# funkelab/cellulus

Hardware: AMD Instinct MI355X
Metric: train crops/sec (U-Net fwd+bwd + OCE loss + Adam) (higher is better)
Workload: dtype f32 (exact 3xbf16 operand split, 6 products, f32 accumulate)

## Files before the change

### cellulus_amd/_clx.py

```python

import ctypes
import os
from ctypes import POINTER, Structure, c_char_p, c_double, c_int, c_longlong, c_size_t, c_void_p

import torch

_HERE = os.path.dirname(os.path.abspath(__file__))
LIB_PATH = os.path.join(_HERE, "libclx.so")


class ClxError(RuntimeError):
    """A libclx entry point returned a negative status."""


class ClxSrc(Structure):

    _fields_ = [
        ("ptr", c_void_p),
        ("C", c_int),
        ("ld", c_int),
        ("D", c_int),
        ("H", c_int),
        ("W", c_int),
        ("oz", c_int),
# ... 6 lines not shown


class ClxPackJob(Structure):

    _fields_ = [("w", c_void_p), ("wp", c_void_p), ("cout", c_int), ("cin", c_int), ("taps", c_int),
                ("cin_pad", c_int), ("cout_pad", c_int), ("mode", c_int)]


class ClxConvDesc(Structure):

    _fields_ = [
        ("nsrc", c_int),
        ("src", ClxSrc * 2),
        ("B", c_int),
        ("ID", c_int),
        ("IH", c_int),
        ("IW", c_int),
        ("KD", c_int),
        ("KH", c_int),
        ("KW", c_int),
        ("PD", c_int),
        ("PH", c_int),
        ("PW", c_int),
        ("N", c_int),
        ("wpack", c_void_p),
        ("bias", c_void_p),
        ("relu", c_int),
        ("mask", c_void_p),
        ("ld_mask", c_int),
        ("out", c_void_p),
        ("ld_out", c_int),
        ("accumulate", c_int),
        ("algo", c_int),
        ("workspace", c_void_p),
        ("workspace_bytes", c_size_t),
        ("vcache", c_void_p),
        ("vcache_valid", c_int),
        ("c_real", c_int),
        ("dy_vcache", c_void_p),
        ("gate_out", c_void_p),
        ("ld_gate", c_int),
        ("mask_bits", c_void_p),
        ("ld_mask_bits", c_int),
        ("det_turns", c_void_p),
        ("adjoint", c_int),
        ("pool_out", c_void_p),
        ("ld_pool", c_int),
        ("tile_list", c_void_p),
        ("tile_count", c_int),
        ("precision", c_int),
        ("wplanes", c_void_p),
        ("aplanes", c_void_p),
        ("aplanes_valid", c_int),
        ("dyplanes", c_void_p),
        ("dyplanes_valid", c_int),
        ("out_planes", c_void_p),
        ("out_colsum", c_void_p),
    ]


_P = c_void_p
_I = c_int
_LL = c_longlong
_D = c_double

PROTOTYPES = {
    "clx_last_error": (c_char_p, []),
    "clx_abi_version": (_I, []),
    "clx_device_count": (_I, []),
    "clx_profile_enable": (_I, [_I]),
    "clx_profile_read": (_I, [_I, POINTER(c_double), POINTER(c_double), POINTER(c_double)]),
    "clx_profile_clock": (_I, [POINTER(c_double), POINTER(c_double), _I]),
    "clx_conv_fwd": (_I, [POINTER(ClxConvDesc), _P]),
    "clx_conv_wgrad": (_I, [POINTER(ClxConvDesc), _P, _I, _P, _P, _P]),
    "clx_chain64_fwd": (_I, [_P, _I, _LL, _P, _P, _P, _I, _P, _I, _P, _P, _I, _I, _P, _I, _P, _I, _P]),
    "clx_chain64_bwd": (_I, [_P, _I, _I, _P, _I, _P, _I, _I, _LL, _P, _P, _P, _I, _P, _P, _P, _P, _P]),
    "clx_pack_weights": (_I, [_P, _P, _I, _I, _I, _I, _I, _I, _P]),
    "clx_pack_weights_batch": (_I, [_P, _I, _LL, _P]),
    "clx_unpack_wgrad": (_I, [_P, _P, _I, _I, _I, _I, _I, _P]),
    "clx_unpack_wgrad_wino": (_I, [_P, _P, _I, _I, _I, _I, _I, _I, _I, _P]),
    "clx_conv_workspace_bytes": (c_size_t, [POINTER(ClxConvDesc), _I]),
    "clx_conv_vcache_bytes": (c_size_t, [POINTER(ClxConvDesc), _I]),
    "clx_conv_sp_covers": (_I, [POINTER(ClxConvDesc), _I]),
    "clx_planes_bytes": (c_size_t, [_LL, _I]),
    "clx_split_planes": (_I, [_P, _LL, _LL, _I, _P, _P]),
    "clx_join_planes": (_I, [_P, _LL, _I, _P, _LL, _P]),
    "clx_gemm_planes": (_I, [_P, _P, _I, _I, _I, _P, _I, _P, _I, _P]),
    "clx_wgrad_planes": (_I, [_P, _P, _LL, _I, _I, _P, _I, _P]),
    "clx_conv_fused_applicable": (_I, [POINTER(ClxConvDesc)]),
    "clx_conv_fused_workspace_bytes": (c_size_t, [POINTER(ClxConvDesc)]),
    "clx_planar_to_pixel": (_I, [_P, _P, _I, _I, _LL, _I, _P]),
    "clx_pixel_to_planar": (_I, [_P, _P, _I, _I, _LL, _I, _P]),
    "clx_depth_to_space": (_I, [_P, _I, _P, _I, _I, _I, _I, _I, _I, _I, _I, _I, _P]),
    "clx_space_to_depth": (_I, [_P, _I, _P, _I, _I, _I, _I, _I, _I, _I, _I, _I, _P]),
    "clx_subpixel_split_weights": (_I, [_P, _P, _P] + [_I] * 10 + [_P]),
    "clx_subpixel_fold_grads": (_I, [_P, _P, _P] + [_I] * 10 + [_P]),
    "clx_maxpool_fwd": (_I, [_P, _P, _I, _I, _I, _I, _I, _I, _I, _I, _P]),
    "clx_changed_rows_workspace": (c_size_t, [_I, _I, _I, _I]),
    "clx_changed_rows": (_I, [_P, _P, _I, _I, _I, _I, _I, _I, _I, _I, _I, _P, _P, _LL, _P, _P]),
    "clx_changed_tiles": (_I, [_P, _I, _I, _I, _I, _I, _I, _I, _I, _I, _I, _I, _P, _P, _LL, _P]),
    "clx_grey_rows": (_I, [_P, _I, _I, _I, _I, _I, _P, _LL, _P, _P, _I, _I, _P, _I, _P]),
    "clx_conv_first_dgrad": (_I, [_P, _I, _P, _I, _I, _I, _I, _I, _I, _I, _P, _P]),
    "clx_gather_rows": (_I, [_P, _I, _P, _LL, _I, _P, _I, _P]),
    "clx_scatter_rows": (_I, [_P, _I, _P, _LL, _I, _P, _I, _P]),
    "clx_broadcast_rows": (_I, [_P, _LL, _P, _I, _P]),
    "clx_maxpool_bwd": (_I, [_P, _P, _P, _P] + [_I] * 7 + [_P] + [_I] * 8 + [_P]),
    "clx_upsample_bwd": (_I, [_P] + [_I] * 8 + [_P, _P] + [_I] * 8 + [_P]),
    "clx_gather_add_fwd": (_I, [_P, _P, _P, _I, _I, _I, _I, _I, _I, _P, _P]),
    "clx_gather_add_bwd": (_I, [_P, _P, _P, _I, _I, _I, _I, _I, _I, _P, _P]),
    "clx_oce_loss_fwd_bwd": (_I, [_P, _P, _P, _P, _LL, _I, ctypes.c_float, ctypes.c_float, ctypes.c_float, _P]),
    "clx_conv_wgrad_turns_bytes": (c_size_t, [POINTER(ClxConvDesc)]),
    "clx_colsum_scratch_bytes": (c_size_t, [_I]),
    "clx_colsum_ordered": (_I, [_P, _I, _LL, _I, _P, _P, _P]),
    "clx_oce_pairs_det_scratch_bytes": (c_size_t, [_I, _I, _LL]),
    "clx_oce_pairs_fused_det": (_I, [_P, _P, _P, _P, _P, _I, _I, _I, _I, _I, _I, ctypes.c_float, ctypes.c_float, _P, _P]),
    "clx_oce_pairs_fused": (_I, [_P, _P, _P, _P, _P, _I, _I, _I, _I, _I, _I, ctypes.c_float, ctypes.c_float, _P]),
    "clx_sample_pairs": (_I, [_P, _P, _P, _I, _I, _I, _I, _I, _I, POINTER(c_int), ctypes.c_ulonglong,
                              ctypes.c_ulonglong, _P]),
    "clx_adam_step": (_I, [_P, _P, _P, _P, _LL, _D, _D, _D, _D, _D, _I, _P]),
    "clx_adam_step_guarded": (_I, [_P, _P, _P, _P, _LL, _D, _D, _D, _D, _D, _I, _P, _P]),
    "clx_noise_stats": (_I, [_P, _P, _I, _I, _LL, _P]),
    "clx_noise_inject": (_I, [_P, _P, _P, _I, _I, _LL, ctypes.c_float, _P]),
    "clx_zero_many": (_I, [POINTER(_P), POINTER(_LL), _I, _P]),
    "clx_gather_rows_f64": (_I, [_P, _P, _LL, _I, _P, _P]),
    "clx_rows_extent_f64": (_I, [_P, _LL, _I, _P, _P]),
    "clx_noise_stats_minmax": (_I, [_P, _P, _I, _I, _LL, _P, _I, _P]),
    "clx_ms_prepare_workspace": (c_size_t, [_LL]),
    "clx_ms_prepare": (_I, [_P, _P, _D, _I, _I, _I, _I, _P, _P, _P, _P, _P]),
    "clx_ms_prepare_f32": (_I, [_P, _P, _D, _I, _I, _I, _I, _P, _P, _P, _P, _P]),
    "clx_ms_iterate": (_I, [_P, _I, _P, _I, _I, _D, _I, _P, _P, _P, _P]),
    "clx_ms_iterate_grid": (_I, [_P, _I, _P, POINTER(c_double), _D, _I, _I, _I, _P, _I, _I, _D, _I,
                                 _P, _P, _P, _P]),
    "clx_ms_assign": (_I, [_P, _P, _I, _P, _I, _I, _P, _P]),
    "clx_ms_assign_grid": (_I, [_P, _P, _I, _P, _I, _I, _P, _P, POINTER(c_double), _D, _I, _I, _I, _P, _P]),
    "clx_ms_assign_cells": (_I, [_P, _P, _I, _P, _I, _I, _P, _P, POINTER(c_double), _D, _I, _I, _I, _P, _P]),
    "clx_ms_assign_dense": (_I, [_P, _P, _I, _I, _P, _P, POINTER(c_double), _D, _I, _I, _I, _P, _I, _I, _I, _I, _P, _P]),
    "clx_ms_dedup_centers": (_I, [_P, _P, _I, _I, _D, _P, POINTER(_I)]),
    "clx_sample_offsets_mt19937": (_I, [_P, POINTER(_I), _I, _I, _LL, _P, POINTER(_I)]),
    "clx_elastic_crop_workspace": (c_size_t, [_I, POINTER(c_int), _I]),
    "clx_elastic_crop": (_I, [_P, _I, _I, _I, _I, POINTER(c_int), POINTER(c_int), POINTER(c_int), ctypes.c_float, _I, _I,
                              _P, _P, _P, _P, _P, _P]),
    "clx_ms_bucket_workspace": (c_size_t, [_I, _LL]),
    "clx_ms_bucket": (_I, [_P, _I, _I, POINTER(c_double), _D, _I, _I, _I, _P, _P, _P, _P]),
    "clx_offset_magnitude": (_I, [_P, _P, _I, _LL, _P]),
    "clx_gaussian_filter_f64": (_I, [_P, _P, _P, _I, _I, _I, _P, _I, _P]),
    "clx_negate_f64": (_I, [_P, _P, _LL, _P]),
    "clx_peak_local_max": (_I, [_P, _I, _I, _I, _P, _P, _I, _P, _P]),
    "clx_greedy_cluster": (_I, [_P, _P, _I, _I, _I, _D, _I, _D, _I, _P, _P, _P, _P]),
    "clx_cc_workspace": (c_size_t, [_LL]),
    "clx_cc_label_filter": (_I, [_P, _P, _I, _I, _I, _I, _P, _P, _P]),
    "clx_edt_workspace": (c_size_t, [_LL]),
    "clx_edt_sq": (_I, [_P, _P, _I, _I, _I, _I, _P, _P]),
    "clx_grow_shrink": (_I, [_P, _I, _I, _I, _I, _I, _P, _P]),
    "clx_minmax_f64": (_I, [_P, _LL, _P, _P]),
    "clx_histogram_f64": (_I, [_P, _LL, _P, _I, _P, _P]),
    "clx_minmax_f32": (_I, [_P, _LL, _P, _P]),
    "clx_histogram_f32": (_I, [_P, _LL, _P, _I, _P, _P]),
    "clx_inst_stats": (_I, [_P, _P, _I, _I, _I, _I, _I, _P, _P, _P]),
    "clx_inst_histogram": (_I, [_P, _P, _I, _LL, _P, _I, _P, _I, _P, _P]),
    "clx_inst_refine": (_I, [_P, _P, _I, _I, _I, _I, _I, _P, _P, _P, _P, _P, _I, _P, _P]),
    "clx_lz4_decompress": (_LL, [_P, _LL, _P, _LL]),
    "clx_blosclz_decompress": (_LL, [_P, _LL, _P, _LL]),
    "clx_blosc_compress_bound": (_LL, [_LL]),
    "clx_blosc_compress_lz4": (_LL, [_P, _LL, _I, _I, _P, _LL]),
    "clx_unshuffle_bytes": (_I, [_P, _P, _LL, _I]),
    "clx_label_presence": (_I, [_P, _LL, _I, _P, _P, _P]),
# ... 90 lines not shown
```

### cellulus_amd/csrc/clx_common.h

```cpp
#pragma once
#include <hip/hip_runtime.h>
#include <hip/hip_ext.h>
#include <stdint.h>
#include <stdio.h>
#include <stdarg.h>
#include "../../include/clx.h"

void clx_set_error(const char* fmt, ...);

#define CLX_REQUIRE(cond, ...)                \
  do {                                        \
    if (!(cond)) {                            \
      clx_set_error(__VA_ARGS__);             \
      return CLX_ERR_ARG;                     \
    }                                         \
  } while (0)

#define CLX_CHECK_LAUNCH(name)                                           \
  do {                                                                   \
    hipError_t e__ = hipGetLastError();                                  \
    if (e__ != hipSuccess) {                                             \
      clx_set_error("%s: launch failed: %s", name, hipGetErrorString(e__)); \
      return CLX_ERR_LAUNCH;                                             \
    }                                                                    \
  } while (0)

typedef float f32x4 __attribute__((ext_vector_type(4)));
typedef float f32x16 __attribute__((ext_vector_type(16)));

struct FastDiv {
  uint32_t m, l, d;
};
static inline FastDiv make_fastdiv(uint32_t d) {
  FastDiv f;
  f.d = d;
  uint32_t l = 0;
  while ((1ull << l) < d) ++l;
  f.l = l;
  f.m = (uint32_t)(((1ull << 32) * ((1ull << l) - d)) / d + 1);
  return f;
}
__device__ __forceinline__ uint32_t fdiv(uint32_t n, const FastDiv& f) {
  return (__umulhi(f.m, n) + n) >> f.l;
}

__device__ __forceinline__ int xcd_remap(int bid, int nblocks) {
  const int q = nblocks >> 3, r = nblocks & 7;
  const int xcd = bid & 7, idx = bid >> 3;
  const int base = (xcd < r) ? xcd * (q + 1) : r * (q + 1) + (xcd - r) * q;
  return base + idx;
}

static inline int cdiv(long long a, long long b) { return (int)((a + b - 1) / b); }

bool clx_smallc_applicable(const clx_conv_desc* d);
int clx_smallc_fwd(const clx_conv_desc* d, hipStream_t st);
int clx_smallc_wgrad(const clx_conv_desc* d, const float* dy, int ld_dy, float* dwpack,
                     float* dbias, hipStream_t st);

int clx_igemm_launch(const clx_conv_desc* d, int batch, long long bs_in, long long bs_w,
                     long long bs_out, hipStream_t st);
int clx_wgrad_launch(const clx_conv_desc* d, const float* dy, int ld_dy, float* dwpack, float* dbias,
                     int batch, long long bs_x, long long bs_dy, long long bs_out, hipStream_t st);
bool clx_sp_fwd_rule(const clx_conv_desc* d);
bool clx_sp_wgrad_rule(const clx_conv_desc* d);
bool clx_sp_applicable(const clx_conv_desc* d);
bool clx_wino_sp(const clx_conv_desc* d);
int clx_sp_launch(const void* A, const void* B, int M, int N, int K, long long rows_a, int batch, long long bs_a, long long bs_b,
                  long long bs_out, const clx_conv_desc* ep, hipStream_t st);
int clx_sp_clock_read(double* shader_ticks, double* wall_ticks, int reset);
int clx_sp_split(const float* x, long long ld, long long rows, int K, void* planes, float* colsum, int nreal, hipStream_t st);
int clx_sp_wgrad_launch(const void* dy_planes, const void* x_planes, long long rows, int N, int C, int batch, long long bs_dy,
                        long long bs_x, long long bs_out, float* dw, int ld_dw, hipStream_t st);
int clx_wino_fwd(const clx_conv_desc* d, hipStream_t st);
int clx_wino_wgrad(const clx_conv_desc* d, const float* dy, int ld_dy, float* dwpack, float* dbias,
                   hipStream_t st);
int clx_wino_pack(const float* w, float* wp, int cout, int cin, int cin_pad, int cout_pad, int dgrad, int tile,
                  int ksize, int kd, hipStream_t st);

int clx_wino_fused_fwd(const clx_conv_desc* d, hipStream_t st);

bool clx_prof_enabled();
void clx_prof_events(int kind, double flops, hipEvent_t* e0, hipEvent_t* e1);
#define CLX_LAUNCH_TIMED(kernel, grid, block, st, e0, e1, ...) \
  hipExtLaunchKernelGGL(kernel, grid, block, 0, st, e0, e1, 0, __VA_ARGS__)
#define CLX_LAUNCH_KIND(kind, kernel, grid, block, lds, st, ...)                              \
  do {                                                                                        \
    hipEvent_t e0__ = nullptr, e1__ = nullptr;                                                \
    if (clx_prof_enabled()) clx_prof_events(kind, 0.0, &e0__, &e1__);                         \
    hipExtLaunchKernelGGL(kernel, grid, block, lds, st, e0__, e1__, 0, __VA_ARGS__);          \
  } while (0)
```

### cellulus_amd/csrc/conv_igemm.hip

```cpp
#include "clx_common.h"
#include <stdlib.h>

#ifdef IG_STAMP
__device__ unsigned long long g_stamps[8 * 32768];
extern "C" int clx_debug_stamps(unsigned long long* host, int n) {
  return hipMemcpyFromSymbol(host, HIP_SYMBOL(g_stamps), sizeof(unsigned long long) * n) == hipSuccess ? 0 : 1;
}
#define STAMP(k) do { if (threadIdx.x == 0 && blockIdx.y == 0 && blockIdx.x < 32768) g_stamps[blockIdx.x * 8 + (k)] = wall_clock64(); } while (0)
#else
#define STAMP(k) do {} while (0)
#endif

__device__ unsigned long long g_clk_ticks[2];
extern "C" int clx_profile_clock(double* shader_ticks, double* wall_ticks_100mhz, int reset) {
  unsigned long long h[2] = {0ull, 0ull};
  if (hipMemcpyFromSymbol(h, HIP_SYMBOL(g_clk_ticks), sizeof(h)) != hipSuccess) {
    clx_set_error("clx_profile_clock: copy failed");
    return CLX_ERR_LAUNCH;
  }
  double sc = 0.0, sw = 0.0;
  if (clx_sp_clock_read(&sc, &sw, reset) != CLX_OK) {
    clx_set_error("clx_profile_clock: copy failed");
    return CLX_ERR_LAUNCH;
  }
// ... 459 lines not shown
          float x = val[j][e];
          if (p.mask) x = (p.mask[(size_t)mrow[j] * p.ld_mask + n + e] > 0.f) ? x : 0.f;
          dst[e] = x;
        }
      }
    }
  }
  STAMP(3);
  if (clk_block) { atomicAdd(&g_clk_ticks[0], clock64() - clk_c0); atomicAdd(&g_clk_ticks[1], wall_clock64() - clk_w0); }
}

}

static const float* zero_buffer() {
  static const float* cache[64] = {nullptr};
  int dev = 0;
  if (hipGetDevice(&dev) != hipSuccess || dev < 0 || dev >= 64) return nullptr;
  if (cache[dev] == nullptr) {
    void* ptr = nullptr;
    if (hipGetSymbolAddress(&ptr, HIP_SYMBOL(g_zero16)) != hipSuccess) return nullptr;
    cache[dev] = (const float*)ptr;
  }
  return cache[dev];
}

static int conv_validate(const clx_conv_desc* d, const char* who) {
  CLX_REQUIRE(d != nullptr, "%s: null descriptor", who);
  CLX_REQUIRE(d->nsrc == 1 || d->nsrc == 2, "%s: nsrc must be 1 or 2", who);
  CLX_REQUIRE(d->B > 0 && d->ID > 0 && d->IH > 0 && d->IW > 0, "%s: bad extent", who);
  const int K[3] = {d->KD, d->KH, d->KW};
  const int P[3] = {d->PD, d->PH, d->PW};
  const int I[3] = {d->ID, d->IH, d->IW};
  for (int i = 0; i < 3; ++i) {
    CLX_REQUIRE(K[i] >= 1 && K[i] <= 3, "%s: kernel extent must be 1, 2 or 3", who);
    CLX_REQUIRE(P[i] >= 0 && P[i] < K[i], "%s: padding must be < kernel extent", who);
    CLX_REQUIRE(I[i] + 2 * P[i] - K[i] + 1 > 0, "%s: input smaller than kernel", who);
  }
  for (int s = 0; s < d->nsrc; ++s) {
    const clx_src& S = d->src[s];
    CLX_REQUIRE(S.ptr != nullptr, "%s: null source %d", who, s);
    CLX_REQUIRE(S.C > 0 && S.C % 4 == 0 && S.ld % 4 == 0 && S.ld >= S.C,
                "%s: source channels/ld must be multiples of 4 (C=%d ld=%d)", who, S.C, S.ld);
    CLX_REQUIRE(((uintptr_t)S.ptr & 15) == 0, "%s: source pointer must be 16-byte aligned", who);
    CLX_REQUIRE(S.fz >= 1 && S.fy >= 1 && S.fx >= 1, "%s: upsample factors >= 1", who);
    CLX_REQUIRE(S.oz >= 0 && S.oy >= 0 && S.ox >= 0, "%s: negative crop", who);
    CLX_REQUIRE((d->ID - 1 + S.oz) / S.fz < S.D && (d->IH - 1 + S.oy) / S.fy < S.H &&
                    (d->IW - 1 + S.ox) / S.fx < S.W,
                "%s: source %d smaller than the logical input", who, s);
  }
  const long long M = (long long)d->B * (d->ID + 2 * d->PD - d->KD + 1) *
                      (d->IH + 2 * d->PH - d->KH + 1) * (d->IW + 2 * d->PW - d->KW + 1);
  CLX_REQUIRE(M < (1ll << 31), "%s: too many output pixels", who);
  return CLX_OK;
}

static void fill_params(const clx_conv_desc* d, ConvP& p) {
  p.nsrc = d->nsrc;
  for (int s = 0; s < 2; ++s) {
    const clx_src& S = d->src[s < d->nsrc ? s : 0];
    p.src[s] = SrcP{S.ptr, S.C, S.ld, S.D, S.H, S.W, S.oz, S.oy, S.ox, S.fz, S.fy, S.fx};
  }
  p.B = d->B; p.ID = d->ID; p.IH = d->IH; p.IW = d->IW;
  p.KD = d->KD; p.KH = d->KH; p.KW = d->KW;
  p.PD = d->PD; p.PH = d->PH; p.PW = d->PW;
  p.OD = d->ID + 2 * d->PD - d->KD + 1;
  p.OH = d->IH + 2 * d->PH - d->KH + 1;
  p.OW = d->IW + 2 * d->PW - d->KW + 1;
  p.N = d->N;
  p.M = d->B * p.OD * p.OH * p.OW;
  p.Ctot = d->src[0].C + (d->nsrc == 2 ? d->src[1].C : 0);
  p.Ktot = p.Ctot * d->KD * d->KH * d->KW;
  p.dOW = make_fastdiv(p.OW); p.dOH = make_fastdiv(p.OH); p.dOD = make_fastdiv(p.OD);
  p.wpack = d->wpack; p.bias = d->bias; p.mask = d->mask; p.out = d->out;
  p.gate_out = d->gate_out; p.ld_gate = d->ld_gate; p.mask_bits = d->mask_bits; p.ld_mask_bits = d->ld_mask_bits;
  p.relu = d->relu; p.ld_mask = d->ld_mask; p.ld_out = d->ld_out;
  p.accumulate = d->accumulate;
  p.bs_in = p.bs_w = p.bs_out = 0;
  p.flush_every = 0;
}

extern "C" int clx_conv_fwd(const clx_conv_desc* d, clx_stream stream) {
  int rc = conv_validate(d, "clx_conv_fwd");
  if (rc) return rc;
  CLX_REQUIRE(d->wpack && d->out, "clx_conv_fwd: null wpack/out");
  CLX_REQUIRE(d->N > 0 && d->ld_out >= d->N, "clx_conv_fwd: bad N/ld_out");
  CLX_REQUIRE(((uintptr_t)d->wpack & 15) == 0, "clx_conv_fwd: wpack must be 16-byte aligned");
  CLX_REQUIRE(d->mask == nullptr || (d->ld_mask >= d->N && d->ld_mask % 4 == 0 &&
                                     ((uintptr_t)d->mask & 15) == 0),
              "clx_conv_fwd: mask must be 16-byte aligned with ld_mask %% 4 == 0 and >= N");
  CLX_REQUIRE(d->ld_out % 4 == 0 && ((uintptr_t)d->out & 15) == 0,
              "clx_conv_fwd: out must be 16-byte aligned with ld_out %% 4 == 0");
  CLX_REQUIRE(d->gate_out == nullptr || (d->relu && d->ld_out % 32 == 0 && d->ld_gate * 32 >= d->ld_out),
              "clx_conv_fwd: gate_out needs relu, ld_out %% 32 == 0 and ld_gate >= ld_out / 32");
  CLX_REQUIRE(d->mask_bits == nullptr || (d->mask == nullptr && d->ld_mask_bits * 32 >= d->N),
              "clx_conv_fwd: mask_bits replaces mask and needs ld_mask_bits >= ceil(N / 32)");
  CLX_REQUIRE(d->algo == CLX_ALGO_DIRECT || d->algo == CLX_ALGO_WINOGRAD || d->algo == CLX_ALGO_WINOGRAD4 ||
                  d->algo == CLX_ALGO_WINOGRAD4_FUSED,
              "clx_conv_fwd: bad algo");
  CLX_REQUIRE((d->out_planes == nullptr && d->out_colsum == nullptr && !d->aplanes_valid) ||
                  (d->algo == CLX_ALGO_DIRECT && d->aplanes != nullptr && clx_sp_applicable(d)),
              "clx_conv_fwd: out_planes / out_colsum / aplanes_valid need the split-precision 1x1 product "
              "(clx_conv_sp_covers, wplanes and aplanes)");
  if (d->algo == CLX_ALGO_WINOGRAD4_FUSED) return clx_wino_fused_fwd(d, (hipStream_t)stream);
  if (d->algo != CLX_ALGO_DIRECT) return clx_wino_fwd(d, (hipStream_t)stream);
  CLX_REQUIRE(d->pool_out == nullptr && d->tile_list == nullptr && !d->adjoint,
              "clx_conv_fwd: pool_out / tile_list / adjoint need a Winograd algorithm (algo = %d)", d->algo);
  if (clx_smallc_applicable(d) && d->mask == nullptr && d->mask_bits == nullptr && d->gate_out == nullptr) {
    clx_smallc_fwd(d, (hipStream_t)stream);
    CLX_CHECK_LAUNCH("clx_conv_fwd(small-channel)");
    return CLX_OK;
  }
  rc = clx_igemm_launch(d, 1, 0, 0, 0, (hipStream_t)stream);
  if (rc) return rc;
  CLX_CHECK_LAUNCH("clx_conv_fwd");
  return CLX_OK;
}

int clx_igemm_launch(const clx_conv_desc* d, int batch, long long bs_in, long long bs_w,
                     long long bs_out, hipStream_t st) {
  if (batch == 1 && d->aplanes != nullptr && clx_sp_applicable(d)) {
    const clx_src& S = d->src[0];
    const long long M = (long long)d->B * d->ID * d->IH * d->IW;
    if (!d->aplanes_valid) {
      const int rc = clx_sp_split(S.ptr, S.ld, M, S.C, d->aplanes, nullptr, 0, st);
      if (rc) return rc;
    }
    return clx_sp_launch(d->aplanes, d->wplanes, (int)M, d->N, S.C, M, 1, 0, 0, 0, d, st);
  }
  ConvP p;
  fill_params(d, p);
  p.zeros = zero_buffer();
  CLX_REQUIRE(p.zeros != nullptr, "clx_conv_fwd: cannot resolve the device zero buffer");
  p.bs_in = bs_in; p.bs_w = bs_w; p.bs_out = bs_out;
  static const int flush_env = getenv("CLX_IGEMM_FLUSH") ? atoi(getenv("CLX_IGEMM_FLUSH")) : 2;
  p.flush_every = flush_env > 0 ? flush_env : 0;
  const bool wide = d->N > 64 && (double)(cdiv(d->N, 128) * 128) / d->N <= 1.2;
  hipEvent_t e0 = nullptr, e1 = nullptr;
  if (clx_prof_enabled())
    clx_prof_events(wide ? CLX_PROF_IGEMM_WIDE : CLX_PROF_IGEMM_NARROW, 2.0 * p.M * p.N * p.Ktot * batch, &e0, &e1);
  static const bool fast_env = getenv("CLX_IGEMM_FAST") == nullptr || atoi(getenv("CLX_IGEMM_FAST")) != 0;
  int fast = fast_env && (long long)p.N * p.Ktot < (1ll << 30) ? 1 : 0;
  const bool padded = d->PD != 0 || d->PH != 0 || d->PW != 0;
  for (int s = 0; s < d->nsrc && fast; ++s) {
    const clx_src& S = d->src[s];
    const long long floats = (long long)d->B * S.D * S.H * S.W * S.ld;
    if (S.C % BK != 0 || floats >= (padded ? (1ll << 29) : (1ll << 30))) fast = 0;
  }
  if (fast && padded) fast = 2;
  static const bool dbg = getenv("CLX_IGEMM_DEBUG") != nullptr;
  if (dbg) fprintf(stderr, "igemm fast=%d wide=%d M=%d N=%d K=%d batch=%d pad=%d%d%d k=%d%d%d nsrc=%d C0=%d\n", (int)fast, (int)wide, p.M, p.N, p.Ktot, batch, d->PD, d->PH, d->PW, d->KD, d->KH, d->KW, d->nsrc, d->src[0].C);
  if (wide) {
    p.nbm = cdiv(p.M, 128); p.nbn = cdiv(p.N, 128);
    if (fast == 1) CLX_LAUNCH_TIMED((conv_igemm_kernel<128, 128, 2, 2, 1>), dim3(p.nbm * p.nbn, batch), dim3(256), st, e0, e1, p);
    else if (fast == 2) CLX_LAUNCH_TIMED((conv_igemm_kernel<128, 128, 2, 2, 2>), dim3(p.nbm * p.nbn, batch), dim3(256), st, e0, e1, p);
    else CLX_LAUNCH_TIMED((conv_igemm_kernel<128, 128, 2, 2>), dim3(p.nbm * p.nbn, batch), dim3(256), st, e0, e1, p);
  } else {
    p.nbm = cdiv(p.M, 128); p.nbn = cdiv(p.N, 64);
    if (fast == 1) CLX_LAUNCH_TIMED((conv_igemm_kernel<128, 64, 4, 1, 1>), dim3(p.nbm * p.nbn, batch), dim3(256), st, e0, e1, p);
    else if (fast == 2) CLX_LAUNCH_TIMED((conv_igemm_kernel<128, 64, 4, 1, 2>), dim3(p.nbm * p.nbn, batch), dim3(256), st, e0, e1, p);
    else CLX_LAUNCH_TIMED((conv_igemm_kernel<128, 64, 4, 1>), dim3(p.nbm * p.nbn, batch), dim3(256), st, e0, e1, p);
  }
  return CLX_OK;
}
```

### cellulus_amd/csrc/conv_smallc.hip

```cpp
#include "clx_common.h"

namespace {

struct SmallP {
  const float* x;
  int ld_x, B, D, H, W;
  int oz, oy, ox;
  int ID, IH, IW, KD, KH, KW, PD, PH, PW, OD, OH, OW;
  int N, M, taps;
  FastDiv dOW, dOH, dOD;
  const float* wpack;
  const float* bias;
  float* out;
  int ld_out, relu;
  const float* dy;
  int ld_dy;
  float* dwp;
  float* dbias;
  int tiles_per_block;
  int RX, items;
  FastDiv dRX;
};

constexpr int PT = 64;
constexpr int MAX_TAPS = 27;

template <int PTILE>
__device__ __forceinline__ void stage_patch(const SmallP& p, int m0, float* Xs) {
  static_assert(256 % PTILE == 0, "a thread keeps one pixel of the tile");
  const int K4 = p.taps;
  const int pl = threadIdx.x % PTILE;
  const uint32_t m = (uint32_t)(m0 + pl);
  const bool live = m < (uint32_t)p.M;
  const uint32_t q1 = fdiv(m, p.dOW);
  const int ox = (int)(m - q1 * p.OW);
  const uint32_t q2 = fdiv(q1, p.dOH);
  const int oy = (int)(q1 - q2 * p.OH);
  const uint32_t q3 = fdiv(q2, p.dOD);
  const int oz = (int)(q2 - q3 * p.OD);
  const int b = (int)q3;
  int tx = 0, ty = 0, tz = 0;
  {
    const int tap = threadIdx.x / PTILE;
    tx = tap % p.KW; ty = (tap / p.KW) % p.KH; tz = tap / (p.KW * p.KH);
  }
  constexpr int STEP = 256 / PTILE;
  for (int tap = threadIdx.x / PTILE; tap < K4; tap += STEP) {
    f32x4 v = {0.f, 0.f, 0.f, 0.f};
    const int lz = oz + tz - p.PD, ly = oy + ty - p.PH, lx = ox + tx - p.PW;
    if (live && (unsigned)lz < (unsigned)p.ID && (unsigned)ly < (unsigned)p.IH && (unsigned)lx < (unsigned)p.IW) {
      const long long pix = (((long long)b * p.D + lz + p.oz) * p.H + ly + p.oy) * p.W + lx + p.ox;
      v = *reinterpret_cast<const f32x4*>(p.x + pix * p.ld_x);
    }
    *reinterpret_cast<f32x4*>(&Xs[(pl * K4 + tap) * 4]) = v;
    tx += STEP;
    while (tx >= p.KW) { tx -= p.KW; if (++ty == p.KH) { ty = 0; ++tz; } }
  }
}

template <int NG>
__global__ __launch_bounds__(256) void conv_smallc_fwd_kernel(const SmallP p) {
  constexpr int PL = 256 / NG;
  constexpr int PPT = PT / PL;
  extern __shared__ float smem[];
  const int K = p.taps * 4;
  float* Ws = smem;
  float* Xs = smem + K * NG * 4;
  const int n0 = blockIdx.y * NG * 4;
  const int ng = threadIdx.x % NG, pl = threadIdx.x / NG;
  __shared__ int used_channels;
  if (threadIdx.x == 0) used_channels = 0;
  __syncthreads();
  int mine_used = 0;
  for (int idx = threadIdx.x; idx < K * NG * 4; idx += 256) {
    const int n = idx / K, k = idx % K;
    const float wv = (n0 + n < p.N) ? p.wpack[(size_t)(n0 + n) * K + k] : 0.f;
    Ws[k * NG * 4 + n] = wv;
    if (wv != 0.f) mine_used |= 1 << (k & 3);
  }
  if (mine_used) atomicOr(&used_channels, mine_used);
  const int n = n0 + ng * 4;
  f32x4 bv = {0.f, 0.f, 0.f, 0.f};
  if (p.bias && n < p.N) {
#pragma unroll
    for (int e = 0; e < 4; ++e) bv[e] = (n + e < p.N) ? p.bias[n + e] : 0.f;
  }
  for (int t = 0; t < p.tiles_per_block; ++t) {
    const int m0 = (blockIdx.x * p.tiles_per_block + t) * PT;
    if (m0 >= p.M) break;
    __syncthreads();
    stage_patch<PT>(p, m0, Xs);
    __syncthreads();
    f32x4 acc[PPT];
#pragma unroll
    for (int i = 0; i < PPT; ++i) acc[i] = bv;
    const int used = used_channels;
    for (int c = 0; c < 4; ++c) {
// ... 85 lines not shown
      }
    } else {
#pragma unroll
      for (int a = 0; a < MT; ++a) {
        if (a < ntap) {
          const int tap = tap0 + a;
          const int lz = oz + tap / (p.KW * p.KH) - p.PD, ly = oy + (tap / p.KW) % p.KH - p.PH, lx = ox + tap % p.KW - p.PW;
          f32x4 xv = {0.f, 0.f, 0.f, 0.f};
          if ((unsigned)lz < (unsigned)p.ID && (unsigned)ly < (unsigned)p.IH && (unsigned)lx < (unsigned)p.IW) {
            const long long pix = (((long long)b * p.D + lz + p.oz) * p.H + ly + p.oy) * p.W + lx + p.ox;
            xv = *reinterpret_cast<const f32x4*>(p.x + pix * p.ld_x);
          }
#pragma unroll
          for (int c = 0; c < 4; ++c) acc[a][c] += xv[c] * dyv;
        }
      }
    }
  }
  __syncthreads();
#pragma unroll
  for (int a = 0; a < MT; ++a) {
    if (a < ntap) {
#pragma unroll
      for (int c = 0; c < 4; ++c)
#pragma unroll
        for (int e = 0; e < 4; ++e) atomicAdd(&red[(a * 4 + c) * NT + g * 4 + e], acc[a][c][e]);
    }
  }
#pragma unroll
  for (int e = 0; e < 4; ++e) atomicAdd(&red[ntap * 4 * NT + g * 4 + e], bsum[e]);
  __syncthreads();
  for (int i = threadIdx.x; i < ntap * 4 * NT; i += 256) {
    const int nl = i % NT, c = (i / NT) & 3, tap = tap0 + i / (4 * NT);
    if (n0 + nl < p.N) atomicAdd(p.dwp + ((size_t)tap * p.N + n0 + nl) * 4 + c, red[i]);
  }
  if (p.dbias && tap0 == 0)
    for (int i = threadIdx.x; i < NT; i += 256)
      if (n0 + i < p.N) atomicAdd(p.dbias + n0 + i, red[ntap * 4 * NT + i]);
}

struct Run {
  int ox0, m0;
  long long base;
};

__device__ __forceinline__ Run decode_run(const SmallP& p, uint32_t item) {
  const uint32_t q1 = fdiv(item, p.dRX);
  const int rx = (int)(item - q1 * p.RX);
  const uint32_t q2 = fdiv(q1, p.dOH);
  const int oy = (int)(q1 - q2 * p.OH);
  const uint32_t q3 = fdiv(q2, p.dOD);
  const int oz = (int)(q2 - q3 * p.OD);
  const int b = (int)q3;
  Run r;
  r.ox0 = rx * 4;
  r.m0 = ((b * p.OD + oz) * p.OH + oy) * p.OW + r.ox0;
  r.base = (((long long)b * p.D + oz + p.oz) * p.H + oy + p.oy) * p.W + r.ox0 + p.ox;
  return r;
}

template <int KD>
struct GreyLane {
  static constexpr int R = KD * 3, NP = R * 6, TAPS = R * 3;
  int px, cq, col;
  long long poff;
  __device__ __forceinline__ GreyLane(const SmallP& p) {
    const int lane = threadIdx.x & 63;
    px = lane >> 4; cq = lane & 15;
    const int l = lane < NP ? lane : 0;
    const int r = l / 6;
    col = l - r * 6;
    const int tz = r / 3, ty = r - tz * 3;
    poff = ((long long)tz * p.H + ty) * p.W;
  }
  __device__ __forceinline__ float load_patch(const SmallP& p, const Run& r) const {
    const int c = r.ox0 + col < p.IW ? col : p.IW - 1 - r.ox0;
    return p.x[(r.base + poff + c) * p.ld_x];
  }
  __device__ __forceinline__ float tap(float pv, int row, int tx) const {
    return __shfl(pv, row * 6 + tx + px, 64);
  }
};

template <int KD>
__global__ __launch_bounds__(256) void conv_grey_fwd_kernel(const SmallP p) {
  using L = GreyLane<KD>;
  const L ln(p);
  const int wave = __builtin_amdgcn_readfirstlane(threadIdx.x >> 6);
  const int n = blockIdx.y * 64 + ln.cq * 4;
  const bool live_n = n < p.N;
  f32x4 w[L::TAPS];
#pragma unroll
  for (int t = 0; t < L::TAPS; ++t)
#pragma unroll
    for (int e = 0; e < 4; ++e) w[t][e] = live_n ? p.wpack[((size_t)(n + e) * L::TAPS + t) * 4] : 0.f;
  f32x4 bv = {0.f, 0.f, 0.f, 0.f};
  if (p.bias && live_n) bv = *reinterpret_cast<const f32x4*>(p.bias + n);
  const uint32_t last = (uint32_t)p.items - 1, stride = gridDim.x * 4;
  uint32_t item = blockIdx.x * 4 + wave;
  Run r[3];
  float pv[3];
#pragma unroll
  for (int s = 0; s < 2; ++s) {
    r[s] = decode_run(p, item + s * stride < last ? item + s * stride : last);
    pv[s] = ln.load_patch(p, r[s]);
  }
  while (true) {
#pragma unroll
    for (int s = 0; s < 3; ++s) {
      if (item > last) return;
      const int s2 = (s + 2) % 3;
      const uint32_t nxt = item + 2 * stride;
      r[s2] = decode_run(p, nxt < last ? nxt : last);
      pv[s2] = ln.load_patch(p, r[s2]);
      f32x4 acc = bv;
#pragma unroll
      for (int row = 0; row < L::R; ++row)
#pragma unroll
        for (int tx = 0; tx < 3; ++tx) acc += ln.tap(pv[s], row, tx) * w[row * 3 + tx];
      if (p.relu) {
#pragma unroll
        for (int e = 0; e < 4; ++e) acc[e] = fmaxf(acc[e], 0.f);
      }
      if (live_n && r[s].ox0 + ln.px < p.OW)
        *reinterpret_cast<f32x4*>(p.out + (size_t)(r[s].m0 + ln.px) * p.ld_out + n) = acc;
      item += stride;
    }
  }
}

template <int KD>
__global__ __launch_bounds__(256) void conv_grey_wgrad_kernel(const SmallP p) {
  using L = GreyLane<KD>;
  __shared__ float red[(L::TAPS + 1) * 64];
  const L ln(p);
  const int wave = __builtin_amdgcn_readfirstlane(threadIdx.x >> 6);
  const int n0 = blockIdx.y * 64, n = n0 + ln.cq * 4;
  const bool live_n = n < p.N;
  const int nld = live_n ? n : 0;
  for (int i = threadIdx.x; i < (L::TAPS + 1) * 64; i += 256) red[i] = 0.f;
  f32x4 acc[L::TAPS];
#pragma unroll
  for (int t = 0; t < L::TAPS; ++t) acc[t] = f32x4{0.f, 0.f, 0.f, 0.f};
  f32x4 bsum = {0.f, 0.f, 0.f, 0.f};
  const uint32_t last = (uint32_t)p.items - 1, stride = gridDim.x * 4;
  uint32_t item = blockIdx.x * 4 + wave;
  auto load_dy = [&](const Run& r) {
    const int m = r.ox0 + ln.px < p.OW ? r.m0 + ln.px : r.m0;
    return *reinterpret_cast<const f32x4*>(p.dy + (size_t)m * p.ld_dy + nld);
  };
  Run r[3];
  float pv[3];
  f32x4 dy[3];
#pragma unroll
  for (int s = 0; s < 2; ++s) {
    r[s] = decode_run(p, item + s * stride < last ? item + s * stride : last);
    pv[s] = ln.load_patch(p, r[s]);
    dy[s] = load_dy(r[s]);
  }
  bool more = item <= last;
  while (more) {
#pragma unroll
    for (int s = 0; s < 3; ++s) {
      if (more) {
        const int s2 = (s + 2) % 3;
        const uint32_t nxt = item + 2 * stride;
        r[s2] = decode_run(p, nxt < last ? nxt : last);
        pv[s2] = ln.load_patch(p, r[s2]);
        dy[s2] = load_dy(r[s2]);
        const bool ok = live_n && r[s].ox0 + ln.px < p.OW;
        f32x4 dyv;
#pragma unroll
        for (int e = 0; e < 4; ++e) dyv[e] = ok ? dy[s][e] : 0.f;
        bsum += dyv;
#pragma unroll
        for (int row = 0; row < L::R; ++row)
#pragma unroll
          for (int tx = 0; tx < 3; ++tx) acc[row * 3 + tx] += ln.tap(pv[s], row, tx) * dyv;
        item += stride;
        more = item <= last;
      }
    }
  }
  __syncthreads();
#pragma unroll
  for (int t = 0; t < L::TAPS; ++t)
#pragma unroll
    for (int e = 0; e < 4; ++e) atomicAdd(&red[t * 64 + ln.cq * 4 + e], acc[t][e]);
#pragma unroll
  for (int e = 0; e < 4; ++e) atomicAdd(&red[L::TAPS * 64 + ln.cq * 4 + e], bsum[e]);
  __syncthreads();
  for (int i = threadIdx.x; i < L::TAPS * 64; i += 256) {
    const int nl = i & 63, t = i >> 6;
    if (n0 + nl < p.N) atomicAdd(p.dwp + ((size_t)t * p.N + n0 + nl) * 4, red[i]);
  }
  if (p.dbias && threadIdx.x < 64 && n0 + threadIdx.x < p.N)
    atomicAdd(p.dbias + n0 + threadIdx.x, red[L::TAPS * 64 + threadIdx.x]);
}

template <int KD>
__global__ __launch_bounds__(256) void conv_grey_rows_kernel(const float* __restrict__ x, int D, int H, int W, int OD,
                                                             int OH, int OW, const int* __restrict__ rows, long long n,
                                                             const float* __restrict__ wpack,
                                                             const float* __restrict__ bias, int relu, int N,
                                                             float* __restrict__ out, int ld_out) {
  constexpr int R = KD * 3, TAPS = R * 3;
  const int lane = threadIdx.x & 63, px = lane >> 4, cq = lane & 15;
  const int nn = blockIdx.y * 64 + cq * 4;
// ... 1 lines not shown
  f32x4 w[TAPS];
#pragma unroll
  for (int t = 0; t < TAPS; ++t)
#pragma unroll
    for (int e = 0; e < 4; ++e) w[t][e] = live_n ? wpack[((size_t)(nn + e) * TAPS + t) * 4] : 0.f;
  f32x4 bv = {0.f, 0.f, 0.f, 0.f};
  if (bias && live_n) bv = *reinterpret_cast<const f32x4*>(bias + nn);
  const long long npo = (long long)OD * OH * OW;
  const long long groups = (n + 3) / 4;
  for (long long g = (long long)blockIdx.x * 4 + (threadIdx.x >> 6); g < groups; g += (long long)gridDim.x * 4) {
    const long long r = g * 4 + px;
    const bool live = r < n;
    const long long row = rows[live ? r : n - 1];
    const long long b = row / npo, pix = row - b * npo;
    const int ox = (int)(pix % OW), oy = (int)((pix / OW) % OH), oz = (int)(pix / ((long long)OW * OH));
    const float* src = x + ((b * D + oz) * H + oy) * (long long)W + ox;
    float xv[TAPS];
#pragma unroll
    for (int rr = 0; rr < R; ++rr)
#pragma unroll
      for (int tx = 0; tx < 3; ++tx) xv[rr * 3 + tx] = src[((long long)(rr / 3) * H + (rr % 3)) * W + tx];
    f32x4 acc = bv;
#pragma unroll
    for (int rr = 0; rr < R; ++rr)
#pragma unroll
      for (int tx = 0; tx < 3; ++tx) acc += xv[rr * 3 + tx] * w[rr * 3 + tx];
    if (relu) {
#pragma unroll
      for (int e = 0; e < 4; ++e) acc[e] = fmaxf(acc[e], 0.f);
    }
    if (live && live_n) *reinterpret_cast<f32x4*>(out + (size_t)r * ld_out + nn) = acc;
  }
}

bool grey_applicable(const clx_conv_desc* d, int ld_act) {
  return d->c_real == 1 && d->KH == 3 && d->KW == 3 && (d->KD == 1 || d->KD == 3) && d->PD == 0 &&
         d->PH == 0 && d->PW == 0 && d->N % 4 == 0 && ld_act % 4 == 0;
}

dim3 grey_grid(SmallP& p) {
  p.RX = cdiv(p.OW, 4);
  p.items = p.B * p.OD * p.OH * p.RX;
  p.dRX = make_fastdiv(p.RX);
  const int ny = cdiv(p.N, 64);
  int nx = 768 / ny;
  if (nx < 1) nx = 1;
  if (nx > cdiv(p.items, 4)) nx = cdiv(p.items, 4);
  return dim3(nx, ny);
}

bool fill(const clx_conv_desc* d, SmallP& p) {
  const clx_src& S = d->src[0];
  p.x = S.ptr; p.ld_x = S.ld; p.B = d->B; p.D = S.D; p.H = S.H; p.W = S.W;
  p.oz = S.oz; p.oy = S.oy; p.ox = S.ox;
  p.ID = d->ID; p.IH = d->IH; p.IW = d->IW;
  p.KD = d->KD; p.KH = d->KH; p.KW = d->KW;
  p.PD = d->PD; p.PH = d->PH; p.PW = d->PW;
  p.OD = d->ID + 2 * d->PD - d->KD + 1;
  p.OH = d->IH + 2 * d->PH - d->KH + 1;
  p.OW = d->IW + 2 * d->PW - d->KW + 1;
  p.N = d->N;
  p.M = d->B * p.OD * p.OH * p.OW;
  p.taps = d->KD * d->KH * d->KW;
  p.dOW = make_fastdiv(p.OW); p.dOH = make_fastdiv(p.OH); p.dOD = make_fastdiv(p.OD);
  return true;
}

int pick_ng(int N) {
  int ng = 4;
  while (ng < 64 && ng * 4 < N) ng *= 2;
  return ng;
}

}

bool clx_smallc_applicable(const clx_conv_desc* d) {
  if (d->nsrc != 1 || d->accumulate) return false;
  const clx_src& S = d->src[0];
  if (S.C != 4 || S.fz != 1 || S.fy != 1 || S.fx != 1) return false;
  const int taps = d->KD * d->KH * d->KW;
  return taps > 1 && taps <= MAX_TAPS && d->N >= 4;
}

int clx_smallc_fwd(const clx_conv_desc* d, hipStream_t st) {
  SmallP p{};
  fill(d, p);
  p.wpack = d->wpack; p.bias = d->bias; p.out = d->out; p.ld_out = d->ld_out; p.relu = d->relu;
  if (grey_applicable(d, d->ld_out) && ((uintptr_t)d->out & 15) == 0 && (!d->bias || ((uintptr_t)d->bias & 15) == 0)) {
    const dim3 grid = grey_grid(p);
    if (d->KD == 1) conv_grey_fwd_kernel<1><<<grid, 256, 0, st>>>(p);
    else conv_grey_fwd_kernel<3><<<grid, 256, 0, st>>>(p);
    return CLX_OK;
  }
  const int ng = pick_ng(p.N);
  const int K = p.taps * 4;
  const int tiles = cdiv(p.M, PT);
  p.tiles_per_block = tiles > 4096 ? 4 : 1;
  const dim3 grid(cdiv(tiles, p.tiles_per_block), cdiv(p.N, ng * 4));
  const size_t lds = (size_t)(K * ng * 4 + PT * K) * sizeof(float);
  switch (ng) {
    case 4: conv_smallc_fwd_kernel<4><<<grid, 256, lds, st>>>(p); break;
    case 8: conv_smallc_fwd_kernel<8><<<grid, 256, lds, st>>>(p); break;
    case 16: conv_smallc_fwd_kernel<16><<<grid, 256, lds, st>>>(p); break;
    case 32: conv_smallc_fwd_kernel<32><<<grid, 256, lds, st>>>(p); break;
    default: conv_smallc_fwd_kernel<64><<<grid, 256, lds, st>>>(p); break;
  }
  return CLX_OK;
}

int clx_smallc_wgrad(const clx_conv_desc* d, const float* dy, int ld_dy, float* dwpack,
                     float* dbias, hipStream_t st) {
  SmallP p{};
  fill(d, p);
  p.dy = dy; p.ld_dy = ld_dy; p.dwp = dwpack; p.dbias = dbias;
  if (grey_applicable(d, ld_dy) && ((uintptr_t)dy & 15) == 0) {
    const dim3 grid = grey_grid(p);
    if (d->KD == 1) conv_grey_wgrad_kernel<1><<<grid, 256, 0, st>>>(p);
    else conv_grey_wgrad_kernel<3><<<grid, 256, 0, st>>>(p);
    return CLX_OK;
  }
  const int ng = pick_ng(p.N);
  const int blocks = p.M < 512 * 64 ? cdiv(p.M, 64) : 512;
  p.tiles_per_block = cdiv(p.M, blocks);
  const dim3 grid(cdiv(p.M, p.tiles_per_block), cdiv(p.N, ng * 4), cdiv(p.taps, 9));
  const size_t lds = (size_t)((p.taps < 9 ? p.taps : 9) * 4 * ng * 4 + ng * 4) * sizeof(float);
  switch (ng) {
    case 4: conv_smallc_wgrad_stream_kernel<4><<<grid, 256, lds, st>>>(p); break;
    case 8: conv_smallc_wgrad_stream_kernel<8><<<grid, 256, lds, st>>>(p); break;
    case 16: conv_smallc_wgrad_stream_kernel<16><<<grid, 256, lds, st>>>(p); break;
    case 32: conv_smallc_wgrad_stream_kernel<32><<<grid, 256, lds, st>>>(p); break;
    default: conv_smallc_wgrad_stream_kernel<64><<<grid, 256, lds, st>>>(p); break;
  }
  return CLX_OK;
}

extern "C" int clx_grey_rows(const float* x, int B, int ID, int IH, int IW, int KD, const int* rows, long long n,
                             const float* wpack, const float* bias, int relu, int N, float* out, int ld_out,
                             clx_stream stream) {
  CLX_REQUIRE(n >= 0, "clx_grey_rows: bad count");
  if (n == 0) return CLX_OK;
  CLX_REQUIRE(x && rows && wpack && out, "clx_grey_rows: null pointer");
  CLX_REQUIRE(B > 0 && (KD == 1 || KD == 3) && ID >= KD && IH >= 3 && IW >= 3, "clx_grey_rows: a 3x3 or 3x3x3 window");
  CLX_REQUIRE(N > 0 && N % 4 == 0 && ld_out % 4 == 0 && ld_out >= N && ((uintptr_t)out & 15) == 0 &&
                  (!bias || ((uintptr_t)bias & 15) == 0),
              "clx_grey_rows: N, ld_out multiples of 4, aligned out / bias");
  const int OD = ID - KD + 1, OH = IH - 2, OW = IW - 2;
  long long gx = (n + 15) / 16;
  if (gx > 4096) gx = 4096;
  const dim3 grid((unsigned)gx, (unsigned)((N + 63) / 64));
  hipStream_t st = (hipStream_t)stream;
  if (KD == 1) conv_grey_rows_kernel<1><<<grid, 256, 0, st>>>(x, ID, IH, IW, OD, OH, OW, rows, n, wpack, bias, relu, N, out, ld_out);
  else conv_grey_rows_kernel<3><<<grid, 256, 0, st>>>(x, ID, IH, IW, OD, OH, OW, rows, n, wpack, bias, relu, N, out, ld_out);
  CLX_CHECK_LAUNCH("clx_grey_rows");
  return CLX_OK;
}
```

### cellulus_amd/csrc/gemm_sp.hip

```cpp
#include "clx_common.h"
#include "sp_planes.h"
#include <stdlib.h>
#include <type_traits>

#ifndef SP_ABL
#define SP_ABL 0
#endif

__device__ unsigned long long g_sp_clk_ticks[2];
int clx_sp_clock_read(double* shader_ticks, double* wall_ticks, int reset) {
  unsigned long long h[2] = {0ull, 0ull};
  if (hipMemcpyFromSymbol(h, HIP_SYMBOL(g_sp_clk_ticks), sizeof(h)) != hipSuccess) return CLX_ERR_LAUNCH;
  *shader_ticks = (double)h[0];
  *wall_ticks = (double)h[1];
  if (reset) {
    const unsigned long long z[2] = {0ull, 0ull};
    if (hipMemcpyToSymbol(HIP_SYMBOL(g_sp_clk_ticks), z, sizeof(z)) != hipSuccess) return CLX_ERR_LAUNCH;
  }
  return CLX_OK;
}

#ifdef SP16_STAMP
__device__ unsigned long long g_sp16_stamps[2][64];
extern "C" int clx_sp16_stamps(unsigned long long* out) {
// ... 116 lines not shown
  const float* mask;
  const unsigned int* mask_bits;
  unsigned int* gate_out;
  const float* zeros;
  int relu, accumulate, ld_out, ld_mask, ld_mask_bits, ld_gate;
  int nbm, nbn;
  char* out_planes;
  float* colsum; int colsum_n;
  unsigned int stride_a, stride_b;
  int total_steps, steps_per_slice, nslices;
};

template <int BM = SP_BM, int NWAVES = 8>
__device__ __forceinline__ void sp_epilogue_from_lds(const SpP& p, const float* Cs, int m0, int n0, int batch, int tid, int lane) {
  constexpr int PASS_ROWS = NWAVES / 4 * 8;
  constexpr int ITERS = BM / PASS_ROWS;
  constexpr int PH = 8;
  const int wv = tid >> 6;
  const int c4 = (wv & 3) * 32 + (lane & 7) * 4;
  const int row0 = (wv >> 2) * 8 + (lane >> 3);
  const int n = n0 + c4;
  const bool n_live = n < p.N;
  f32x4 csum = {0.f, 0.f, 0.f, 0.f};
  const long long prow = p.out_planes ? sp::padded_rows(p.M) : 0;
#pragma unroll 1
  for (int h0 = 0; h0 < ITERS; h0 += PH) {
    f32x4 val[PH];
    int mrow[PH];
    bool live[PH];
#pragma unroll
    for (int j = 0; j < PH; ++j) {
      const int row = row0 + PASS_ROWS * (h0 + j);
      mrow[j] = m0 + row;
      live[j] = mrow[j] < p.M && n_live;
      val[j] = *reinterpret_cast<const f32x4*>(&Cs[row * LDC + c4]);
    }
    float* const out_base = p.out + batch * p.bs_out + n;
    if (p.accumulate) {
      f32x4 prev[PH];
#pragma unroll
      for (int j = 0; j < PH; ++j)
        prev[j] = *reinterpret_cast<const f32x4*>(live[j] ? out_base + (size_t)mrow[j] * p.ld_out : p.zeros);
#pragma unroll
      for (int j = 0; j < PH; ++j) val[j] += prev[j];
    }
    if (p.relu) {
#pragma unroll
      for (int j = 0; j < PH; ++j)
#pragma unroll
        for (int e = 0; e < 4; ++e) val[j][e] = fmaxf(val[j][e], 0.f);
    }
    if (p.mask_bits) {
      unsigned int wd[PH];
#pragma unroll
      for (int j = 0; j < PH; ++j) wd[j] = live[j] ? p.mask_bits[(size_t)mrow[j] * p.ld_mask_bits + (n >> 5)] : 0u;
#pragma unroll
      for (int j = 0; j < PH; ++j)
#pragma unroll
        for (int e = 0; e < 4; ++e) val[j][e] = ((wd[j] >> ((n & 31) + e)) & 1u) ? val[j][e] : 0.f;
    }
    if (p.gate_out) {
#pragma unroll
      for (int j = 0; j < PH; ++j) {
        unsigned int nib = 0u;
#pragma unroll
        for (int e = 0; e < 4; ++e) nib |= (live[j] && val[j][e] > 0.f) ? (1u << e) : 0u;
        unsigned int word = nib << (4 * (lane & 7));
        word |= __shfl_xor(word, 1, 64);
        word |= __shfl_xor(word, 2, 64);
        word |= __shfl_xor(word, 4, 64);
        if ((lane & 7) == 0 && mrow[j] < p.M && n < p.ld_out) p.gate_out[(size_t)mrow[j] * p.ld_gate + (n >> 5)] = word;
      }
    }
    if (p.mask) {
      f32x4 mk[PH];
#pragma unroll
      for (int j = 0; j < PH; ++j)
        mk[j] = *reinterpret_cast<const f32x4*>(live[j] ? p.mask + (size_t)mrow[j] * p.ld_mask + n : p.zeros);
#pragma unroll
      for (int j = 0; j < PH; ++j)
#pragma unroll
        for (int e = 0; e < 4; ++e) val[j][e] = (!live[j] || mk[j][e] > 0.f) ? val[j][e] : 0.f;
    }
#pragma unroll
    for (int j = 0; j < PH; ++j)
      if (live[j]) *reinterpret_cast<f32x4*>(out_base + (size_t)mrow[j] * p.ld_out) = val[j];
    if (p.out_planes) {
#pragma unroll
      for (int j = 0; j < PH; ++j)
        if (n_live && mrow[j] < prow)
          sp::store4(p.out_planes, mrow[j], n, p.N >> 4, live[j] ? val[j] : f32x4{0.f, 0.f, 0.f, 0.f});
    }
    if (p.colsum) {
#pragma unroll
      for (int j = 0; j < PH; ++j)
        if (live[j]) csum += val[j];
    }
  }
  if (p.colsum) {
#pragma unroll
    for (int e = 0; e < 4; ++e) {
      csum[e] += __shfl_xor(csum[e], 8, 64);
      csum[e] += __shfl_xor(csum[e], 16, 64);
      csum[e] += __shfl_xor(csum[e], 32, 64);
    }
    if ((lane >> 3) == 0 && n_live) {
#pragma unroll
      for (int e = 0; e < 4; ++e)
        if (n + e < p.colsum_n) atomicAdd(p.colsum + n + e, csum[e]);
    }
  }
}

template <int MODE>
__global__ __launch_bounds__(512, 1) void gemm_sp_kernel(const SpP p) {
  __shared__ __attribute__((aligned(16))) char smem[RING * STAGE];
  const int tid = threadIdx.x, lane = tid & 63;
  const int w = __builtin_amdgcn_readfirstlane(tid >> 6);
  const int wm = w >> 1, wn = w & 1;
  int tile_m, tile_n, batch, step0 = 0, ksteps;
  if constexpr (MODE == 0) {
    const int v = xcd_remap(blockIdx.x, p.nbm * p.nbn);
    tile_n = v % p.nbn; tile_m = v / p.nbn;
    batch = blockIdx.y;
    ksteps = p.ksteps;
  } else {
    const int T = p.nbm * p.nbn;
    const int u = xcd_remap(blockIdx.x, gridDim.x);
    const int per_batch = T * p.nslices;
    batch = u / per_batch;
    const int v = u % per_batch;
    const int slice = v / T, t = v % T;
    tile_n = t % p.nbn; tile_m = t / p.nbn;
    step0 = slice * p.steps_per_slice;
    ksteps = p.total_steps - step0 < p.steps_per_slice ? p.total_steps - step0 : p.steps_per_slice;
  }
  const int m0 = tile_m * SP_BM, n0 = tile_n * SP_BN;
  const bool clk_block = blockIdx.x == gridDim.x / 2 && blockIdx.y == gridDim.y / 2 && threadIdx.x == 0;
  unsigned long long clk_c0 = 0, clk_w0 = 0;
  if (clk_block) { clk_c0 = clock64(); clk_w0 = wall_clock64(); }

  const char* const Ab = p.A + batch * p.bs_a;
  const char* const Bb = p.B + batch * p.bs_b;
  auto frag_base = [&](int f) __attribute__((always_inline)) -> const char* {
    if constexpr (MODE == 0) {
      if (f < A_FRAGS) {
        int rb = tile_m * (SP_BM / 32) + f / 3;
        if (rb > p.rb_a - 1) rb = p.rb_a - 1;
        return Ab + ((long long)rb * ksteps * 3 + f % 3) * FRAG;
      }
      const int g = f - A_FRAGS;
      const int nb = tile_n * (SP_BN / 32) + g / 3;
      return Bb + ((long long)nb * ksteps * 3 + g % 3) * FRAG;
    } else {
      if (f < A_FRAGS) {
        int cb = tile_m * (SP_BM / 32) + f / 3;
        if (cb > p.M / 32 - 1) cb = p.M / 32 - 1;
        return Ab + ((long long)(2 * cb) * 3 + f % 3) * FRAG;
      }
      const int g = f - A_FRAGS;
      const int cb = tile_n * (SP_BN / 32) + g / 3;
      return Bb + ((long long)(2 * cb) * 3 + g % 3) * FRAG;
    }
  };
  const char* gsrc[5];
#pragma unroll
  for (int q = 0; q < 4; ++q) gsrc[q] = frag_base(w + 8 * q);
  gsrc[4] = frag_base(32 + (w & 3));
  const int l_oct = lane >> 4, l_pix = (lane & 15) ^ (4 * (lane >> 4));
// ... 789 lines not shown
  CLX_REQUIRE(x != nullptr && planes != nullptr, "clx_split_planes: null pointer");
  CLX_REQUIRE(rows > 0 && K > 0 && K % 16 == 0 && ld >= K && ld % 4 == 0, "clx_split_planes: K must be a multiple of 16, ld >= K a multiple of 4");
  CLX_REQUIRE(((uintptr_t)x & 15) == 0 && ((uintptr_t)planes & 15) == 0, "clx_split_planes: pointers must be 16-byte aligned");
  const int ksteps = K / 16;
  const long long nfrag = sp::padded_rows(rows) / 32 * ksteps;
  long long blocks = (nfrag + 3) / 4;
  if (blocks > 8192) blocks = 8192;
  if (colsum != nullptr) {
    if (blocks > 2048) blocks = 2048;
    int g = ksteps % 4 == 0 ? 4 : ksteps % 2 == 0 ? 2 : 1;
    const long long unit = ksteps / g;
    blocks = (blocks + unit - 1) / unit * unit;
    CLX_LAUNCH_KIND(CLX_PROF_SPLIT_PLANES, sp_split_kernel<true>, dim3((unsigned)blocks), dim3(256), 0, st, x, ld, rows, ksteps, (char*)planes,
                    nfrag, colsum, nreal);
  } else {
    CLX_LAUNCH_KIND(CLX_PROF_SPLIT_PLANES, sp_split_kernel<false>, dim3((unsigned)blocks), dim3(256), 0, st, x, ld, rows, ksteps, (char*)planes,
                    nfrag, (float*)nullptr, 0);
  }
  return CLX_OK;
}

extern "C" int clx_split_planes(const float* x, long long ld, long long rows, int K, void* planes, clx_stream stream) {
  const int rc = clx_sp_split(x, ld, rows, K, planes, nullptr, 0, (hipStream_t)stream);
  if (rc) return rc;
  CLX_CHECK_LAUNCH("clx_split_planes");
  return CLX_OK;
}

extern "C" int clx_join_planes(const void* planes, long long rows, int K, float* x, long long ld, clx_stream stream) {
  CLX_REQUIRE(x != nullptr && planes != nullptr, "clx_join_planes: null pointer");
  CLX_REQUIRE(rows > 0 && K > 0 && K % 16 == 0 && ld >= K, "clx_join_planes: K must be a multiple of 16, ld >= K");
  const long long nfrag = sp::padded_rows(rows) / 32 * (K / 16);
  long long blocks = (nfrag + 3) / 4;
  if (blocks > 8192) blocks = 8192;
  sp_join_kernel<<<dim3((unsigned)blocks), dim3(256), 0, (hipStream_t)stream>>>((const char*)planes, ld, rows, K / 16, x, nfrag);
  CLX_CHECK_LAUNCH("clx_join_planes");
  return CLX_OK;
}

static bool sp_pointwise(const clx_conv_desc* d) {
  if (d->precision != CLX_PREC_F32X3BF16 || d->nsrc != 1) return false;
  if (d->KD != 1 || d->KH != 1 || d->KW != 1 || d->PD || d->PH || d->PW) return false;
  const clx_src& S = d->src[0];
  if (S.fz != 1 || S.fy != 1 || S.fx != 1 || S.oz || S.oy || S.ox) return false;
  return S.D == d->ID && S.H == d->IH && S.W == d->IW;
}

bool clx_sp_fwd_rule(const clx_conv_desc* d) {
  return sp_pointwise(d) && d->N % SP_BN == 0 && d->src[0].C % 64 == 0 && d->src[0].C >= 128 && d->ld_out % 4 == 0;
}

bool clx_sp_wgrad_rule(const clx_conv_desc* d) {
  if (!sp_pointwise(d) || d->N % 128 != 0 || d->src[0].C % 128 != 0) return false;
  const long long ch = d->N > d->src[0].C ? d->N : d->src[0].C;
  return (long long)d->B * d->ID * d->IH * d->IW * ch * 6 < (1ll << 32) - (1 << 24);
}

bool clx_sp_applicable(const clx_conv_desc* d) { return d->wplanes != nullptr && clx_sp_fwd_rule(d); }

extern "C" int clx_conv_sp_covers(const clx_conv_desc* d, int pass) {
  if (d == nullptr || (pass != CLX_PASS_FWD && pass != CLX_PASS_WGRAD)) return 0;
  if (d->algo == CLX_ALGO_WINOGRAD || d->algo == CLX_ALGO_WINOGRAD4) return clx_wino_sp(d) ? 1 : 0;
  if (d->algo != CLX_ALGO_DIRECT) return 0;
  return (pass == CLX_PASS_FWD ? clx_sp_fwd_rule(d) : clx_sp_wgrad_rule(d)) ? 1 : 0;
}

int clx_sp_launch(const void* A, const void* B, int M, int N, int K, long long rows_a, int batch, long long bs_a, long long bs_b,
                  long long bs_out, const clx_conv_desc* ep, hipStream_t st) {
  CLX_REQUIRE(M > 0 && N > 0 && N % SP_BN == 0 && K >= 128 && K % 64 == 0, "clx_gemm_planes: needs N %% 128 == 0, K %% 64 == 0 and K >= 128");
  CLX_REQUIRE(rows_a >= M, "clx_gemm_planes: the A planes hold fewer rows than M");
  SpP p = {};
  p.A = (const char*)A; p.B = (const char*)B;
  p.bs_a = bs_a; p.bs_b = bs_b; p.bs_out = bs_out;
  p.out = ep->out; p.ld_out = ep->ld_out;
  p.M = M; p.N = N; p.ksteps = K / 16;
  p.rb_a = (int)(sp::padded_rows(rows_a) / 32);
  p.bias = ep->bias; p.mask = ep->mask; p.mask_bits = ep->mask_bits; p.gate_out = ep->gate_out;
  p.relu = ep->relu; p.accumulate = ep->accumulate; p.ld_mask = ep->ld_mask; p.ld_mask_bits = ep->ld_mask_bits; p.ld_gate = ep->ld_gate;
  p.zeros = sp_zero_buffer();
  CLX_REQUIRE(p.zeros != nullptr, "clx_gemm_planes: cannot resolve the device zero buffer");
  p.out_planes = batch == 1 ? (char*)ep->out_planes : nullptr;
  p.colsum = batch == 1 ? ep->out_colsum : nullptr; p.colsum_n = N;
  CLX_REQUIRE(p.out_planes == nullptr || ep->ld_out == N, "clx_gemm_planes: out_planes needs a dense output (ld_out == N)");
  p.nbm = cdiv(M, SP_BM); p.nbn = N / SP_BN;
  const char* const tile_env = getenv("CLX_SP_TILE");
  const int tile_choice = tile_env != nullptr ? atoi(tile_env) : 0;
  const char* const maxk_env = getenv("CLX_SP_TILE_MAXK");
  const int maxk = maxk_env != nullptr ? atoi(maxk_env) : 1024;
  const bool small_tiles = tile_choice == 128 || (tile_choice != 256 && K <= maxk);
  const char* const shape_env = getenv("CLX_SP_MFMA");
  const bool mfma16 = shape_env != nullptr && atoi(shape_env) == 16;
  hipEvent_t e0 = nullptr, e1 = nullptr;
  if (clx_prof_enabled())
    clx_prof_events(small_tiles && !mfma16 ? CLX_PROF_GEMM_SP2 : CLX_PROF_GEMM_SP, 2.0 * M * N * K * batch, &e0, &e1);
  if (mfma16) CLX_LAUNCH_TIMED(gemm_sp16_kernel, dim3(p.nbm * p.nbn, batch), dim3(512), st, e0, e1, p);
  else if (small_tiles) CLX_LAUNCH_TIMED(gemm_sp2_kernel, dim3(cdiv(M, S2_BM) * (N / S2_BN), batch), dim3(256), st, e0, e1, p);
  else CLX_LAUNCH_TIMED(gemm_sp_kernel<0>, dim3(p.nbm * p.nbn, batch), dim3(512), st, e0, e1, p);
  return CLX_OK;
}

int clx_sp_wgrad_launch(const void* dy_planes, const void* x_planes, long long rows, int N, int C, int batch, long long bs_dy,
                        long long bs_x, long long bs_out, float* dw, int ld_dw, hipStream_t st) {
  CLX_REQUIRE(rows > 0 && N > 0 && C > 0 && N % 128 == 0 && C % 128 == 0, "clx_wgrad_planes: needs N %% 128 == 0 and C %% 128 == 0");
  SpP p = {};
  p.A = (const char*)dy_planes; p.B = (const char*)x_planes;
  p.bs_a = bs_dy; p.bs_b = bs_x; p.bs_out = bs_out;
  p.out = dw; p.ld_out = ld_dw;
  p.M = N; p.N = C;
  p.stride_a = (unsigned int)(N / 16) * KSTEP; p.stride_b = (unsigned int)(C / 16) * KSTEP;
  CLX_REQUIRE(sp::planes_bytes(rows, N) < (1ll << 32) && sp::planes_bytes(rows, C) < (1ll << 32), "clx_wgrad_planes: operand planes beyond 4 GB");
  p.total_steps = (int)(sp::padded_rows(rows) / 16);
  p.nbm = cdiv(N, SP_BM); p.nbn = C / SP_BN;
  const int tiles = p.nbm * p.nbn * batch;
  int cus = 256, dev = 0;
  if (hipGetDevice(&dev) == hipSuccess) (void)hipDeviceGetAttribute(&cus, hipDeviceAttributeMultiprocessorCount, dev);
  int best_ns = 1;
  double best = 1e30;
  const int max_ns = p.total_steps / 8 > 0 ? p.total_steps / 8 : 1;
  for (int ns = 1; ns <= max_ns && ns <= 4096; ++ns) {
    const int sps = (cdiv(p.total_steps, ns) + 7) / 8 * 8;
    const int real_ns = cdiv(p.total_steps, sps);
    if (p.total_steps - (real_ns - 1) * sps < 8) continue;
    const double cost = (double)cdiv((long long)tiles * real_ns, cus) * (sps + 12);
    if (cost < best) { best = cost; best_ns = ns; }
    if ((long long)tiles * ns > 16ll * cus) break;
  }
  p.steps_per_slice = (cdiv(p.total_steps, best_ns) + 7) / 8 * 8;
  p.nslices = cdiv(p.total_steps, p.steps_per_slice);
  CLX_REQUIRE(p.total_steps >= 8 && p.total_steps - (p.nslices - 1) * p.steps_per_slice >= 8, "clx_wgrad_planes: internal: a slice of fewer than 8 steps");
  hipEvent_t e0 = nullptr, e1 = nullptr;
  if (clx_prof_enabled()) clx_prof_events(CLX_PROF_WGRAD_SP, 2.0 * rows * N * C * batch, &e0, &e1);
  CLX_LAUNCH_TIMED(gemm_sp_kernel<1>, dim3(p.nbm * p.nbn * p.nslices * batch), dim3(512), st, e0, e1, p);
  return CLX_OK;
}

extern "C" int clx_wgrad_planes(const void* dy_planes, const void* x_planes, long long rows, int N, int C, float* dw, int ld_dw,
                                clx_stream stream) {
  CLX_REQUIRE(dy_planes && x_planes && dw && ld_dw >= C, "clx_wgrad_planes: null pointer / ld_dw < C");
  const int rc = clx_sp_wgrad_launch(dy_planes, x_planes, rows, N, C, 1, 0, 0, 0, dw, ld_dw, (hipStream_t)stream);
  if (rc) return rc;
  CLX_CHECK_LAUNCH("clx_wgrad_planes");
  return CLX_OK;
}

extern "C" int clx_gemm_planes(const void* a_planes, const void* b_planes, int M, int N, int K, const float* bias, int relu,
                               float* out, int ld_out, clx_stream stream) {
  CLX_REQUIRE(a_planes && b_planes && out, "clx_gemm_planes: null pointer");
  CLX_REQUIRE(ld_out >= N && ld_out % 4 == 0 && ((uintptr_t)out & 15) == 0, "clx_gemm_planes: out must be 16-byte aligned, ld_out %% 4 == 0");
  clx_conv_desc ep = {};
  ep.out = out; ep.ld_out = ld_out; ep.bias = bias; ep.relu = relu;
  const int rc = clx_sp_launch(a_planes, b_planes, M, N, K, M, 1, 0, 0, 0, &ep, (hipStream_t)stream);
  if (rc) return rc;
  CLX_CHECK_LAUNCH("clx_gemm_planes");
  return CLX_OK;
}
```

### cellulus_amd/csrc/wino.hip

```cpp
#include "clx_common.h"
#include "sp_planes.h"
#include "wino_tables.h"

namespace {

inline int grid_for(long long total, int block) {
  long long g = (total + block - 1) / block;
  if (g > 16384) g = 16384;
  if (g < 1) g = 1;
  return (int)g;
}

__device__ __forceinline__ f32x4 ld4(const float* p) { return *reinterpret_cast<const f32x4*>(p); }
__device__ __forceinline__ void st4(float* p, f32x4 v) { *reinterpret_cast<f32x4*>(p) = v; }

struct Geom {
  int B, SH, SW, oy, ox;
  int ID, SD, oz;
  int IH, IW, P;
  int OH, OW, th, tw;
  long long T;
};

template <int MT, int R, bool PL = false>
__global__ __launch_bounds__(256) void wino_input_kernel(const float* __restrict__ x, int ld_x, int C4, Geom g,
                                                         float* __restrict__ V, long long total,
                                                         const int* __restrict__ tile_list = nullptr, long long Tc = 0,
                                                         long long plane_bytes = 0) {
  using W = WT<MT, R>;
  constexpr int A = W::A;
  const int C = C4 * 4;
  const long long Trows = tile_list ? Tc : g.T;
  const long long plane = Trows * C;
  for (long long i = (long long)blockIdx.x * blockDim.x + threadIdx.x; i < total;
       i += (long long)gridDim.x * blockDim.x) {
    int c;
    long long t;
    if constexpr (PL) {
      sp::item_to_row_channel(i, C, t, c);
      if (t >= Trows) continue;
    } else {
      c = (int)(i % C4) * 4;
      t = i / C4;
    }
    const long long tg = tile_list ? (long long)tile_list[t] : t;
    const int tx = (int)(tg % g.tw);
    const long long q = tg / g.tw;
    const int ty = (int)(q % g.th);
    const int b = (int)(q / g.th);
    const int bb = b / g.ID, bz = b - bb * g.ID;
    f32x4 d[A][A];
#pragma unroll
    for (int r = 0; r < A; ++r) {
      const int ly = MT * ty - g.P + r;
#pragma unroll
      for (int s = 0; s < A; ++s) {
        const int lx = MT * tx - g.P + s;
        f32x4 v = {0.f, 0.f, 0.f, 0.f};
        if ((unsigned)ly < (unsigned)g.IH && (unsigned)lx < (unsigned)g.IW) {
          const long long pix = (((long long)bb * g.SD + bz + g.oz) * g.SH + ly + g.oy) * g.SW + lx + g.ox;
          v = ld4(x + pix * ld_x + c);
        }
        d[r][s] = v;
      }
    }
    f32x4 w[A][A];
#pragma unroll
    for (int s = 0; s < A; ++s)
#pragma unroll
      for (int r = 0; r < A; ++r) {
        f32x4 acc = {0.f, 0.f, 0.f, 0.f};
        bool first = true;
#pragma unroll
        for (int k = 0; k < A; ++k) axpy(acc, first, W::BT[r][k], d[k][s]);
        w[r][s] = acc;
      }
    float* dst = V + t * C + c;
#pragma unroll
    for (int r = 0; r < A; ++r)
#pragma unroll
      for (int qq = 0; qq < A; ++qq) {
        f32x4 acc = {0.f, 0.f, 0.f, 0.f};
        bool first = true;
#pragma unroll
        for (int k = 0; k < A; ++k) axpy(acc, first, W::BT[qq][k], w[r][k]);
        if constexpr (PL) sp::store4(reinterpret_cast<char*>(V) + (r * A + qq) * plane_bytes, t, c, C >> 4, acc);
        else st4(dst + (r * A + qq) * plane, acc);
      }
  }
}

template <int MT, int R>
__global__ __launch_bounds__(256) void wino_output_kernel(const float* __restrict__ M, int N4, Geom g,
                                                          const float* __restrict__ bias, int relu,
                                                          const float* __restrict__ mask, int ld_mask,
                                                          float* __restrict__ out, int ld_out, int Nreal,
                                                          int accumulate, unsigned int* __restrict__ gate_out,
                                                          int ld_gate, const unsigned int* __restrict__ mask_bits,
                                                          int ld_mask_bits, float* __restrict__ pool_out, int ld_pool,
                                                          long long total, const int* __restrict__ tile_list = nullptr,
                                                          long long Tc = 0) {
  using W = WT<MT, R>;
  constexpr int A = W::A;
  constexpr int MP = MT / 2;
  const int N = N4 * 4;
  const long long plane = (tile_list ? Tc : g.T) * N;
  const int sub = threadIdx.x & 7;
  for (long long i = (long long)blockIdx.x * blockDim.x + threadIdx.x; i < total;
       i += (long long)gridDim.x * blockDim.x) {
    const int n = (int)(i % N4) * 4;
    const long long t = i / N4;
    const long long tg = tile_list ? (long long)tile_list[t] : t;
    const int tx = (int)(tg % g.tw);
    const long long q = tg / g.tw;
    const int ty = (int)(q % g.th);
    const int b = (int)(q / g.th);
    const float* src = M + t * N + n;
    f32x4 rr[MT][A];
#pragma unroll
    for (int s = 0; s < A; ++s) {
      f32x4 m[A];
#pragma unroll
      for (int k = 0; k < A; ++k) m[k] = ld4(src + (k * A + s) * plane);
#pragma unroll
      for (int a = 0; a < MT; ++a) {
        f32x4 acc = {0.f, 0.f, 0.f, 0.f};
        bool first = true;
#pragma unroll
        for (int k = 0; k < A; ++k) axpy(acc, first, W::AT[a][k], m[k]);
        rr[a][s] = acc;
      }
    }
    f32x4 bv = {0.f, 0.f, 0.f, 0.f};
    if (bias) {
#pragma unroll
      for (int e = 0; e < 4; ++e) bv[e] = (n + e < Nreal) ? bias[n + e] : 0.f;
    }
    f32x4 pm[MP][MP];
#pragma unroll
    for (int a = 0; a < MT; ++a) {
      const int oy = MT * ty + a;
      if (oy >= g.OH) continue;
#pragma unroll
      for (int cc = 0; cc < MT; ++cc) {
        const int ox = MT * tx + cc;
        if (ox >= g.OW) continue;
        f32x4 v = {0.f, 0.f, 0.f, 0.f};
        bool first = true;
#pragma unroll
        for (int k = 0; k < A; ++k) axpy(v, first, W::AT[cc][k], rr[a][k]);
        v += bv;
        const long long m = ((long long)b * g.OH + oy) * g.OW + ox;
        if (accumulate) {
          v += ld4(out + m * ld_out + n);
        }
        if (relu) {
#pragma unroll
          for (int e = 0; e < 4; ++e) v[e] = fmaxf(v[e], 0.f);
        }
        if (mask_bits) {
          const unsigned int wbits = mask_bits[m * ld_mask_bits + (n >> 5)] >> (n & 31);
#pragma unroll
          for (int e = 0; e < 4; ++e) v[e] = ((wbits >> e) & 1u) ? v[e] : 0.f;
        }
        if (gate_out) {
          unsigned int nib = 0u;
#pragma unroll
          for (int e = 0; e < 4; ++e) nib |= (n + e < Nreal && v[e] > 0.f) ? (1u << e) : 0u;
          unsigned int word = nib << (4 * sub);
          word |= __shfl_xor(word, 1, 64);
          word |= __shfl_xor(word, 2, 64);
          word |= __shfl_xor(word, 4, 64);
          if (sub == 0) gate_out[m * ld_gate + (n >> 5)] = word;
        }
        if (n + 3 < Nreal) {
          if (mask) {
            const f32x4 mk = ld4(mask + m * ld_mask + n);
#pragma unroll
            for (int e = 0; e < 4; ++e) v[e] = (mk[e] > 0.f) ? v[e] : 0.f;
          }
          st4(out + m * ld_out + n, v);
        } else {
          for (int e = 0; e < 4 && n + e < Nreal; ++e) {
            float xv = v[e];
            if (mask) xv = (mask[m * ld_mask + n + e] > 0.f) ? xv : 0.f;
            out[m * ld_out + n + e] = xv;
          }
        }
        if (pool_out) {
          if ((a & 1) == 0 && (cc & 1) == 0) pm[a >> 1][cc >> 1] = v;
          else {
#pragma unroll
            for (int e = 0; e < 4; ++e) pm[a >> 1][cc >> 1][e] = fmaxf(pm[a >> 1][cc >> 1][e], v[e]);
          }
          if ((a & 1) && (cc & 1)) {
            const long long pm_ = ((long long)b * (g.OH >> 1) + (oy >> 1)) * (g.OW >> 1) + (ox >> 1);
            st4(pool_out + pm_ * ld_pool + n, pm[a >> 1][cc >> 1]);
          }
        }
      }
    }
  }
}

constexpr int ADJ_SEG = 8;

__global__ __launch_bounds__(256) void wino_adjoint_output_kernel(const float* __restrict__ Pm, int C4, int Bn, int th,
                                                                  int tw, int IH, int IW, const float* __restrict__ mask,
                                                                  int ld_mask, const unsigned int* __restrict__ mask_bits,
                                                                  int ld_mask_bits, float* __restrict__ out, int ld_out,
                                                                  int Creal, long long total) {
  using W = WT<4, 3>;
  constexpr int A = 6;
  const int C = C4 * 4;
  const int bh = (IH + 3) / 4, bw = (IW + 3) / 4;
  const int nseg = (bh + ADJ_SEG - 1) / ADJ_SEG;
  const long long plane = (long long)Bn * th * tw * C;
  for (long long i = (long long)blockIdx.x * blockDim.x + threadIdx.x; i < total;
       i += (long long)gridDim.x * blockDim.x) {
    const int c = (int)(i % C4) * 4;
    long long t = i / C4;
    const int bx = (int)(t % bw);
    long long q = t / bw;
    const int sg = (int)(q % nseg);
    const int b = (int)(q / nseg);
    const int by0 = sg * ADJ_SEG, by1 = min(by0 + ADJ_SEG, bh);
    f32x4 carry[2][4];
#pragma unroll
    for (int a = 0; a < 2; ++a)
#pragma unroll
      for (int e = 0; e < 4; ++e) carry[a][e] = f32x4{0.f, 0.f, 0.f, 0.f};
    for (int ty = by0 - 1; ty < by1; ++ty) {
      f32x4 d[A][4];
#pragma unroll
      for (int a = 0; a < A; ++a)
#pragma unroll
        for (int e = 0; e < 4; ++e) d[a][e] = f32x4{0.f, 0.f, 0.f, 0.f};
      if (ty >= 0 && ty < th) {
#pragma unroll
        for (int ux = 0; ux < 2; ++ux) {
          const int tx = bx - ux;
          if (tx < 0 || tx >= tw) continue;
          const float* src = Pm + (((long long)b * th + ty) * tw + tx) * C + c;
#pragma unroll
          for (int s2 = 0; s2 < A; ++s2) {
            f32x4 pcol[A], wcol[A];
#pragma unroll
            for (int r = 0; r < A; ++r) pcol[r] = ld4(src + (r * A + s2) * plane);
#pragma unroll
            for (int a = 0; a < A; ++a) {
              f32x4 v = {0.f, 0.f, 0.f, 0.f};
              bool first = true;
#pragma unroll
              for (int r = 0; r < A; ++r) axpy(v, first, W::BT[r][a], pcol[r]);
              wcol[a] = v;
            }
#pragma unroll
            for (int e = 0; e < 4; ++e) {
              if (ux && e >= 2) continue;
              const float coef = ux ? W::BT[s2][4 + (e & 1)] : W::BT[s2][e];
#pragma unroll
              for (int a = 0; a < A; ++a) {
                bool first = false;
                axpy(d[a][e], first, coef, wcol[a]);
              }
            }
          }
        }
      }
      if (ty >= by0) {
#pragma unroll
        for (int a = 0; a < 4; ++a) {
          const int y = 4 * ty + a;
          if (y >= IH) continue;
#pragma unroll
          for (int e = 0; e < 4; ++e) {
            const int x = 4 * bx + e;
            if (x >= IW) continue;
            f32x4 v = d[a][e];
            if (a < 2) v += carry[a][e];
            const long long m = ((long long)b * IH + y) * IW + x;
            if (mask_bits) {
              const unsigned int wbits = mask_bits[m * ld_mask_bits + (c >> 5)] >> (c & 31);
#pragma unroll
              for (int k = 0; k < 4; ++k) v[k] = ((wbits >> k) & 1u) ? v[k] : 0.f;
            }
            if (c + 3 < Creal) {
              if (mask) {
                const f32x4 mk = ld4(mask + m * ld_mask + c);
#pragma unroll
                for (int k = 0; k < 4; ++k) v[k] = (mk[k] > 0.f) ? v[k] : 0.f;
              }
              st4(out + m * ld_out + c, v);
            } else {
              for (int k = 0; k < 4 && c + k < Creal; ++k) {
                float xv = v[k];
                if (mask) xv = (mask[m * ld_mask + c + k] > 0.f) ? xv : 0.f;
                out[m * ld_out + c + k] = xv;
              }
            }
          }
        }
      }
#pragma unroll
      for (int e = 0; e < 4; ++e) { carry[0][e] = d[4][e]; carry[1][e] = d[5][e]; }
    }
  }
}

template <int MT, int R, bool PL = false>
__global__ __launch_bounds__(256) void wino_dy_kernel(const float* __restrict__ dy, int ld_dy, int N4,
                                                      Geom g, float* __restrict__ Md,
                                                      float* __restrict__ dbias, int Nreal,
                                                      long long total, long long plane_bytes = 0) {
  using W = WT<MT, R>;
  constexpr int A = W::A;
  extern __shared__ float bacc[];
  const int N = N4 * 4;
  const long long plane = g.T * N;
  if (dbias) {
    for (int k = threadIdx.x; k < N; k += blockDim.x) bacc[k] = 0.f;
    __syncthreads();
  }
  for (long long i = (long long)blockIdx.x * blockDim.x + threadIdx.x; i < total;
       i += (long long)gridDim.x * blockDim.x) {
    int n;
    long long t;
    if constexpr (PL) {
      sp::item_to_row_channel(i, N, t, n);
      if (t >= g.T) continue;
    } else {
      n = (int)(i % N4) * 4;
      t = i / N4;
    }
    const int tx = (int)(t % g.tw);
    const long long q = t / g.tw;
    const int ty = (int)(q % g.th);
    const int b = (int)(q / g.th);
    f32x4 d[MT][MT];
    f32x4 sum = {0.f, 0.f, 0.f, 0.f};
#pragma unroll
    for (int a = 0; a < MT; ++a)
#pragma unroll
      for (int c = 0; c < MT; ++c) {
        const int oy = MT * ty + a, ox = MT * tx + c;
        f32x4 v = {0.f, 0.f, 0.f, 0.f};
        if (oy < g.OH && ox < g.OW) v = ld4(dy + (((long long)b * g.OH + oy) * g.OW + ox) * ld_dy + n);
        d[a][c] = v;
        sum += v;
      }
    if (dbias) {
#pragma unroll
      for (int e = 0; e < 4; ++e) atomicAdd(&bacc[n + e], sum[e]);
    }
    f32x4 w[A][MT];
#pragma unroll
    for (int c = 0; c < MT; ++c)
#pragma unroll
      for (int r = 0; r < A; ++r) {
        f32x4 acc = {0.f, 0.f, 0.f, 0.f};
        bool first = true;
#pragma unroll
        for (int a = 0; a < MT; ++a) axpy(acc, first, W::AT[a][r], d[a][c]);
        w[r][c] = acc;
      }
    float* dst = Md + t * N + n;
#pragma unroll
    for (int r = 0; r < A; ++r)
#pragma unroll
      for (int qq = 0; qq < A; ++qq) {
        f32x4 acc = {0.f, 0.f, 0.f, 0.f};
        bool first = true;
#pragma unroll
        for (int c = 0; c < MT; ++c) axpy(acc, first, W::AT[c][qq], w[r][c]);
        if constexpr (PL) sp::store4(reinterpret_cast<char*>(Md) + (r * A + qq) * plane_bytes, t, n, N >> 4, acc);
        else st4(dst + (r * A + qq) * plane, acc);
      }
  }
  if (dbias) {
    __syncthreads();
    for (int k = threadIdx.x; k < Nreal; k += blockDim.x)
      if (bacc[k] != 0.f) atomicAdd(dbias + k, bacc[k]);
  }
}

template <int MT, int R, bool PL = false>
__global__ __launch_bounds__(256) void wino_dy_dual_kernel(const float* __restrict__ dy, int ld_dy, int N4,
                                                           Geom gd, Geom gw, float* __restrict__ Vd,
// ... 274 lines not shown
inline int pad4(int n) { return (n + 3) / 4 * 4; }

inline bool wino_sp(const clx_conv_desc* d) {
  if (d->precision != CLX_PREC_F32X3BF16 || d->KD != 1 || d->ID != 1 || d->N % 128 != 0 || d->src[0].C % 128 != 0) return false;
  const int mt = d->algo == CLX_ALGO_WINOGRAD ? 2 : 4;
  const long long eh = d->IH + (d->PH ? d->KH - 1 : 0), ew = d->IW + (d->PW ? d->KW - 1 : 0);
  const long long tiles = (long long)d->B * ((eh + mt - 1) / mt) * ((ew + mt - 1) / mt);
  const int ch = d->N > d->src[0].C ? d->N : d->src[0].C;
  return sp::planes_bytes(tiles, ch) < (1ll << 32);
}
inline long long sp_items(long long rows, int C) { return (rows + 7) / 8 * 8 * (C / 4); }

clx_conv_desc gemm_desc(float* V, int C, const clx_conv_desc* d, const Geom& gin) {
  clx_conv_desc gd = {};
  gd.nsrc = 1;
  gd.src[0].ptr = V; gd.src[0].C = C; gd.src[0].ld = C;
  gd.src[0].D = d->ID; gd.src[0].H = 1; gd.src[0].W = gin.th * gin.tw;
  gd.src[0].fz = gd.src[0].fy = gd.src[0].fx = 1;
  gd.B = d->B; gd.ID = d->ID; gd.IH = 1; gd.IW = gin.th * gin.tw;
  gd.KD = d->KD; gd.KH = gd.KW = 1;
  gd.PD = d->PD;
  return gd;
}

template <int MT, int R>
int wino_fwd_t(const clx_conv_desc* d, hipStream_t st) {
  constexpr int AA = WT<MT, R>::A * WT<MT, R>::A;
  const Geom gin = geom(d, MT, d->ID), gout = geom(d, MT, out_planes(d));
  const clx_src& S = d->src[0];
  const int C = S.C, Np = pad4(d->N);
  const bool spx = wino_sp(d);
  CLX_REQUIRE(!spx || d->wplanes != nullptr, "clx_conv_fwd(winograd): precision f32x3bf16 needs wplanes (the planes of wpack)");
  float* V = d->vcache ? (float*)d->vcache : (float*)d->workspace;
  const int* list = d->tile_list;
  if (list != nullptr) {
    CLX_REQUIRE(d->KD == 1 && d->ID == 1 && d->PH == 0 && d->vcache == nullptr && !d->accumulate && d->tile_count >= 0 &&
                    d->tile_count <= gin.T && gin.T == gout.T,
                "clx_conv_fwd(winograd): tile_list needs a 2-D valid convolution without vcache / accumulate and at most "
                "th * tw * B tiles");
    if (d->tile_count == 0) return CLX_OK;
  }
  const long long Tin = list ? d->tile_count : gin.T, Tout = list ? d->tile_count : gout.T;
  const long long pbV = spx ? sp::planes_bytes(Tin, C) : 0;
  float* M = spx ? (float*)((char*)d->workspace + AA * sp::planes_bytes(gin.T, C)) : (float*)d->workspace + AA * Tin * C;
  if (!(d->vcache && d->vcache_valid)) {
    if (spx) {
      const long long tot_in = sp_items(Tin, C);
      int rc = clx_sp_zero_tail(V, Tin, C, AA, pbV, st);
      if (rc) return rc;
      CLX_LAUNCH_KIND(CLX_PROF_WINO_TRANSFORM, (wino_input_kernel<MT, R, true>), dim3(grid_for(tot_in, 256)), dim3(256), 0, st, S.ptr, S.ld, C / 4,
                      gin, V, tot_in, list, Tin, pbV);
    } else {
      const long long tot_in = Tin * (C / 4);
      CLX_LAUNCH_KIND(CLX_PROF_WINO_TRANSFORM, (wino_input_kernel<MT, R>), dim3(grid_for(tot_in, 256)), dim3(256), 0, st, S.ptr, S.ld, C / 4, gin, V,
                      tot_in, list, Tin, 0ll);
    }
  }
  if (spx) {
    clx_conv_desc ep = {};
    ep.out = M; ep.ld_out = Np;
    const int rc = clx_sp_launch(V, d->wplanes, (int)Tin, d->N, C, Tin, AA, pbV, sp::planes_bytes(Np, C), Tout * Np, &ep, st);
    if (rc) return rc;
  } else {
    clx_conv_desc gd = gemm_desc(V, C, d, gin);
    if (list) {
      gd.B = 1;
      gd.src[0].W = gd.IW = (int)Tin;
    }
    gd.N = d->N; gd.wpack = d->wpack; gd.out = M; gd.ld_out = Np;
    const int rc = clx_igemm_launch(&gd, AA, Tin * C, (long long)Np * d->KD * C, Tout * Np, st);
    if (rc) return rc;
  }
  const long long tot_out = Tout * (Np / 4);
  CLX_REQUIRE((d->gate_out == nullptr && d->mask_bits == nullptr) || Np % 32 == 0,
              "clx_conv_fwd(winograd): gate_out / mask_bits need a channel count that is a multiple of 32");
  CLX_REQUIRE(d->gate_out == nullptr || d->relu, "clx_conv_fwd(winograd): gate_out needs relu");
  if (d->pool_out != nullptr) {
    CLX_REQUIRE(d->KD == 1 && d->ID == 1 && gout.OH % 2 == 0 && gout.OW % 2 == 0,
                "clx_conv_fwd(winograd): pool_out needs a 2-D layer with even output height and width");
    CLX_REQUIRE(d->N % 4 == 0 && d->ld_pool % 4 == 0 && d->ld_pool >= d->N && ((uintptr_t)d->pool_out & 15) == 0 &&
                    d->mask == nullptr && d->mask_bits == nullptr && !d->accumulate,
                "clx_conv_fwd(winograd): pool_out needs N %% 4 == 0, an aligned ld_pool >= N, and no mask / accumulate");
  }
  CLX_LAUNCH_KIND(CLX_PROF_WINO_TRANSFORM, (wino_output_kernel<MT, R>), dim3(grid_for(tot_out, 256)), dim3(256), 0, st, M, Np / 4, gout, d->bias,
                  d->relu, d->mask, d->ld_mask, d->out, d->ld_out, d->N, d->accumulate, d->gate_out, d->ld_gate, d->mask_bits,
                  d->ld_mask_bits, d->pool_out, d->ld_pool, tot_out, list, Tout);
  CLX_CHECK_LAUNCH("clx_conv_fwd(winograd)");
  return CLX_OK;
}

template <int MT, int R>
int wino_wgrad_t(const clx_conv_desc* d, const float* dy, int ld_dy, float* dwpack, float* dbias, hipStream_t st) {
  constexpr int AA = WT<MT, R>::A * WT<MT, R>::A;
  const Geom gin = geom(d, MT, d->ID), gout = geom(d, MT, out_planes(d));
  const clx_src& S = d->src[0];
  const int C = S.C, N = d->N;
  const bool spx = wino_sp(d);
  float* V = d->vcache ? (float*)d->vcache : (float*)d->workspace;
  const long long pbV = spx ? sp::planes_bytes(gin.T, C) : 0, pbM = spx ? sp::planes_bytes(gout.T, N) : 0;
  float* Md = spx ? (float*)((char*)d->workspace + AA * pbV) : (float*)d->workspace + AA * gin.T * C;
  if (!(d->vcache && d->vcache_valid)) {
    if (spx) {
      const long long tot_in = sp_items(gin.T, C);
      int rc = clx_sp_zero_tail(V, gin.T, C, AA, pbV, st);
      if (rc) return rc;
      CLX_LAUNCH_KIND(CLX_PROF_WINO_TRANSFORM, (wino_input_kernel<MT, R, true>), dim3(grid_for(tot_in, 256)), dim3(256), 0, st, S.ptr, S.ld, C / 4,
                      gin, V, tot_in, (const int*)nullptr, 0ll, pbV);
    } else {
      const long long tot_in = gin.T * (C / 4);
      CLX_LAUNCH_KIND(CLX_PROF_WINO_TRANSFORM, (wino_input_kernel<MT, R>), dim3(grid_for(tot_in, 256)), dim3(256), 0, st, S.ptr, S.ld, C / 4, gin, V,
                      tot_in, (const int*)nullptr, 0ll, 0ll);
    }
  }
  if (spx) {
    const int rc = clx_sp_zero_tail(Md, gout.T, N, AA, pbM, st);
    if (rc) return rc;
  }
  if (d->dy_vcache) {
    Geom gd = gout;
    gd.SH = gout.OH; gd.SW = gout.OW; gd.oy = gd.ox = 0;
    gd.ID = gd.SD = out_planes(d); gd.oz = 0;
    gd.IH = gout.OH; gd.IW = gout.OW; gd.P = R - 1;
    gd.OH = gout.OH + R - 1; gd.OW = gout.OW + R - 1;
    gd.th = (gd.OH + MT - 1) / MT; gd.tw = (gd.OW + MT - 1) / MT;
    gd.T = (long long)gd.B * gd.th * gd.tw;
    const long long tot = spx ? sp_items(gd.T, N) : gd.T * (N / 4);
    int blocks = grid_for(tot, 256);
    if (dbias && blocks > 2048) blocks = 2048;
    if (spx) {
      const long long pbD = sp::planes_bytes(gd.T, N);
      const int rc = clx_sp_zero_tail(d->dy_vcache, gd.T, N, AA, pbD, st);
      if (rc) return rc;
      CLX_LAUNCH_KIND(CLX_PROF_WINO_TRANSFORM, (wino_dy_dual_kernel<MT, R, true>), dim3(blocks), dim3(256), (size_t)N * sizeof(float), st, dy, ld_dy,
                      N / 4, gd, gout, (float*)d->dy_vcache, Md, dbias, N, tot, pbD, pbM);
    } else {
      CLX_LAUNCH_KIND(CLX_PROF_WINO_TRANSFORM, (wino_dy_dual_kernel<MT, R>), dim3(blocks), dim3(256), (size_t)N * sizeof(float), st, dy, ld_dy, N / 4,
                      gd, gout, (float*)d->dy_vcache, Md, dbias, N, tot, 0ll, 0ll);
    }
  } else {
    const long long tot_dy = spx ? sp_items(gout.T, N) : gout.T * (N / 4);
    int blocks = grid_for(tot_dy, 256);
    if (blocks > 2048) blocks = 2048;
    if (spx)
      CLX_LAUNCH_KIND(CLX_PROF_WINO_TRANSFORM, (wino_dy_kernel<MT, R, true>), dim3(blocks), dim3(256), (size_t)N * sizeof(float), st, dy, ld_dy, N / 4,
                      gout, Md, dbias, N, tot_dy, pbM);
    else
      CLX_LAUNCH_KIND(CLX_PROF_WINO_TRANSFORM, (wino_dy_kernel<MT, R>), dim3(blocks), dim3(256), (size_t)N * sizeof(float), st, dy, ld_dy, N / 4, gout,
                      Md, dbias, N, tot_dy, 0ll);
  }
  if (spx) {
    CLX_REQUIRE(gin.T == gout.T, "clx_conv_wgrad(winograd): tile counts of input and output differ");
    CLX_REQUIRE(d->det_turns == nullptr, "clx_conv_wgrad: the reproducible mode exists for the float32 precision only");
    const int rc = clx_sp_wgrad_launch(Md, V, gin.T, N, C, AA, pbM, pbV, (long long)N * C, dwpack, C, st);
    if (rc) return rc;
    CLX_CHECK_LAUNCH("clx_conv_wgrad(winograd, split precision)");
    return CLX_OK;
  }
  clx_conv_desc gd = gemm_desc(V, C, d, gin);
  gd.N = N;
  gd.det_turns = d->det_turns;
  const int rc = clx_wgrad_launch(&gd, Md, N, dwpack, nullptr, AA, gin.T * C, gout.T * N,
                                  (long long)d->KD * N * C, st);
  if (rc) return rc;
  CLX_CHECK_LAUNCH("clx_conv_wgrad(winograd)");
  return CLX_OK;
}

}

bool clx_wino_sp(const clx_conv_desc* d) { return wino_sp(d); }

extern "C" size_t clx_conv_workspace_bytes(const clx_conv_desc* d, int pass) {
  if (d == nullptr || !applicable(d)) return 0;
  if (pass == CLX_PASS_WGRAD && d->PH != 0) return 0;
  const int mt = tile_of(d), a = mt + d->KH - 1;
  const Geom gin = geom(d, mt, d->ID), gout = geom(d, mt, out_planes(d));
  if (gout.OH <= 0 || gout.OW <= 0 || out_planes(d) <= 0 || gin.T >= (1ll << 31) || gout.T >= (1ll << 31)) return 0;
  const long long C = d->src[0].C, N = pad4(d->N);
  if (wino_sp(d)) {
    const long long v = sp::planes_bytes(gin.T, (int)C);
    const long long m = pass == CLX_PASS_WGRAD ? sp::planes_bytes(gout.T, (int)N) : gout.T * N * (long long)sizeof(float);
    return (size_t)(a * a * (v + m));
  }
  return (size_t)(a * a * (gin.T * C + gout.T * N)) * sizeof(float);
}

extern "C" size_t clx_conv_vcache_bytes(const clx_conv_desc* d, int which) {
  if (d == nullptr || !applicable(d)) return 0;
  const int mt = tile_of(d), a = mt + d->KH - 1, R = d->KH;
  const Geom gin = geom(d, mt, d->ID), gout = geom(d, mt, out_planes(d));
  const long long C = d->src[0].C, N = pad4(d->N);
  if (which == 0) return wino_sp(d) ? (size_t)(a * a * sp::planes_bytes(gin.T, (int)C)) : (size_t)(a * a * gin.T * C) * sizeof(float);
  const long long th = (gout.OH + R - 1 + mt - 1) / mt, tw = (gout.OW + R - 1 + mt - 1) / mt;
  const long long Td = (long long)gout.B * th * tw;
  return wino_sp(d) ? (size_t)(a * a * sp::planes_bytes(Td, (int)N)) : (size_t)(a * a * Td * N) * sizeof(float);
}

static int wino_adjoint(const clx_conv_desc* d, hipStream_t st) {
  CLX_REQUIRE(d->algo == CLX_ALGO_WINOGRAD4 && d->KH == 3 && d->KW == 3 && d->PH == 2 && d->PW == 2 && d->nsrc == 1 &&
                  ((d->KD == 1 && d->ID == 1 && d->PD == 0) || (d->KD == 3 && d->PD == 2)),
              "clx_conv_fwd(adjoint): a 3x3 (2-D) or 3x3x3 layer in its data-gradient form (padding 2) with "
              "CLX_ALGO_WINOGRAD4 only");
  CLX_REQUIRE(d->bias == nullptr && !d->relu && !d->accumulate && d->gate_out == nullptr,
              "clx_conv_fwd(adjoint): only the ReLU-gate epilogues (mask / mask_bits) exist");
  CLX_REQUIRE(d->N % 4 == 0 && d->src[0].C % 4 == 0, "clx_conv_fwd(adjoint): channel counts must be multiples of 4");
  const int OHf = d->IH, OWf = d->IW;
  const int th = (OHf + 3) / 4, tw = (OWf + 3) / 4;
  const int planes_dy = d->ID, planes_dx = d->ID + 2 * d->PD - (d->KD - 1);
  const long long Tdy = (long long)d->B * planes_dy * th * tw, Tdx = (long long)d->B * planes_dx * th * tw;
  const int Nf = d->src[0].C, Cp = d->N;
  const bool spx = wino_sp(d);
  const size_t need = spx ? (size_t)36 * (sp::planes_bytes(Tdx, Cp) + sp::planes_bytes(Tdy, Nf))
                          : (size_t)36 * (Tdx * Cp + Tdy * Nf) * sizeof(float);
  CLX_REQUIRE(d->workspace != nullptr && d->workspace_bytes >= need && ((uintptr_t)d->workspace & 15) == 0,
              "clx_conv_fwd(adjoint): needs the %zu workspace bytes of the layer's weight gradient (%zu given)", need,
              d->workspace_bytes);
  CLX_REQUIRE(d->mask_bits == nullptr || Cp % 32 == 0, "clx_conv_fwd(adjoint): mask_bits needs whole words per pixel");
  float* P = (float*)d->workspace;
  float* Mdy = P + (size_t)36 * Tdx * Cp;
  if (spx) {
    CLX_REQUIRE(d->wplanes != nullptr, "clx_conv_fwd(adjoint): precision f32x3bf16 needs wplanes");
    const char* Mp = (const char*)d->workspace + 36 * sp::planes_bytes(Tdx, Cp);
    clx_conv_desc ep = {};
    ep.out = P; ep.ld_out = Cp;
    const int rc = clx_sp_launch(Mp, d->wplanes, (int)Tdy, Cp, Nf, Tdy, 36, sp::planes_bytes(Tdy, Nf), sp::planes_bytes(Cp, Nf),
                                 Tdx * Cp, &ep, st);
    if (rc) return rc;
  } else {
  clx_conv_desc gd = {};
  gd.nsrc = 1;
  gd.src[0].ptr = Mdy; gd.src[0].C = Nf; gd.src[0].ld = Nf;
  gd.src[0].D = planes_dy; gd.src[0].H = 1; gd.src[0].W = th * tw;
  gd.src[0].fz = gd.src[0].fy = gd.src[0].fx = 1;
  gd.B = d->B; gd.ID = planes_dy; gd.IH = 1; gd.IW = th * tw;
  gd.KD = d->KD; gd.KH = gd.KW = 1; gd.PD = d->PD;
  gd.N = Cp; gd.wpack = d->wpack; gd.out = P; gd.ld_out = Cp;
  const int rc = clx_igemm_launch(&gd, 36, Tdy * Nf, (long long)Cp * d->KD * Nf, Tdx * Cp, st);
  if (rc) return rc;
  }
  const int IH = OHf + 2, IW = OWf + 2;
  const int nseg = ((IH + 3) / 4 + ADJ_SEG - 1) / ADJ_SEG;
  const long long total = (long long)d->B * planes_dx * nseg * ((IW + 3) / 4) * (Cp / 4);
  CLX_LAUNCH_KIND(CLX_PROF_WINO_TRANSFORM, wino_adjoint_output_kernel, dim3(grid_for(total, 256)), dim3(256), 0, st, P, Cp / 4,
                  d->B * planes_dx, th, tw, IH, IW, d->mask, d->ld_mask, d->mask_bits, d->ld_mask_bits, d->out, d->ld_out, Cp, total);
  CLX_CHECK_LAUNCH("clx_conv_fwd(winograd adjoint)");
  return CLX_OK;
}

int clx_wino_fwd(const clx_conv_desc* d, hipStream_t st) {
  if (d->adjoint) return wino_adjoint(d, st);
  CLX_REQUIRE(applicable(d), "clx_conv_fwd: Winograd does not apply to this geometry");
  const size_t need = clx_conv_workspace_bytes(d, CLX_PASS_FWD);
  CLX_REQUIRE(d->workspace != nullptr && d->workspace_bytes >= need && need > 0,
              "clx_conv_fwd: Winograd needs %zu workspace bytes (%zu given)", need, d->workspace_bytes);
  CLX_REQUIRE(((uintptr_t)d->workspace & 15) == 0 && ((uintptr_t)d->vcache & 15) == 0,
              "clx_conv_fwd: workspace / vcache must be 16-byte aligned");
  if (d->KH == 2) return wino_fwd_t<4, 2>(d, st);
  return tile_of(d) == 4 ? wino_fwd_t<4, 3>(d, st) : wino_fwd_t<2, 3>(d, st);
}

int clx_wino_wgrad(const clx_conv_desc* d, const float* dy, int ld_dy, float* dwpack, float* dbias,
                   hipStream_t st) {
  CLX_REQUIRE(applicable(d) && d->PH == 0, "clx_conv_wgrad: Winograd does not apply to this geometry");
  const size_t need = clx_conv_workspace_bytes(d, CLX_PASS_WGRAD);
  CLX_REQUIRE(d->workspace != nullptr && d->workspace_bytes >= need && need > 0,
              "clx_conv_wgrad: Winograd needs %zu workspace bytes (%zu given)", need, d->workspace_bytes);
  CLX_REQUIRE(((uintptr_t)d->workspace & 15) == 0 && ((uintptr_t)d->vcache & 15) == 0,
              "clx_conv_wgrad: workspace / vcache must be 16-byte aligned");
  CLX_REQUIRE(d->N <= 8192, "clx_conv_wgrad: too many output channels for the Winograd bias accumulator");
  if (d->KH == 2) return wino_wgrad_t<4, 2>(d, dy, ld_dy, dwpack, dbias, st);
  return tile_of(d) == 4 ? wino_wgrad_t<4, 3>(d, dy, ld_dy, dwpack, dbias, st)
                         : wino_wgrad_t<2, 3>(d, dy, ld_dy, dwpack, dbias, st);
}

int clx_wino_pack(const float* w, float* wp, int cout, int cin, int cin_pad, int cout_pad, int dgrad,
                  int tile, int ksize, int kd, hipStream_t st) {
  const bool fused = dgrad == 3;
  if (fused) dgrad = 0;
  const int rows = dgrad ? cin_pad : cout_pad, cols = dgrad ? cout_pad : cin_pad;
  const long long total = (long long)rows * kd * cols;
  const int grid = grid_for(total, 256);
  if (ksize == 2) wino_filter_kernel<4, 2><<<grid, 256, 0, st>>>(w, wp, cout, cin, rows, cols, kd, dgrad, total, fused);
  else if (tile == 4) wino_filter_kernel<4, 3><<<grid, 256, 0, st>>>(w, wp, cout, cin, rows, cols, kd, dgrad, total, fused);
  else wino_filter_kernel<2, 3><<<grid, 256, 0, st>>>(w, wp, cout, cin, rows, cols, kd, dgrad, total, fused);
  return CLX_OK;
}

extern "C" int clx_pack_weights_batch(const clx_pack_job* jobs, int njobs, long long max_total, clx_stream stream) {
  CLX_REQUIRE(jobs != nullptr && njobs > 0 && njobs < 65536 && max_total > 0, "clx_pack_weights_batch: bad arguments");
  CLX_REQUIRE(((uintptr_t)jobs & 7) == 0, "clx_pack_weights_batch: the job table must be 8-byte aligned");
  long long gx = (max_total + 255) / 256;
  if (gx > 512) gx = 512;
  pack_batch_kernel<<<dim3((unsigned)gx, (unsigned)njobs), 256, 0, (hipStream_t)stream>>>(jobs);
  CLX_CHECK_LAUNCH("clx_pack_weights_batch");
  return CLX_OK;
}

extern "C" int clx_unpack_wgrad_wino(const float* du, float* dw, int cout, int cin, int rows,
                                     int cin_pad, int tile, int ksize, int kd, clx_stream stream) {
  CLX_REQUIRE(du && dw, "clx_unpack_wgrad_wino: null pointer");
  CLX_REQUIRE(cout > 0 && cin > 0 && rows >= cout && cin_pad >= cin, "clx_unpack_wgrad_wino: bad extents");
  CLX_REQUIRE((ksize == 3 && (tile == 2 || tile == 4)) || (ksize == 2 && tile == 4),
              "clx_unpack_wgrad_wino: (tile, ksize) must be (2, 3), (4, 3) or (4, 2)");
  CLX_REQUIRE(kd == 1 || (kd == ksize && tile == 4), "clx_unpack_wgrad_wino: kd must be 1 or ksize (F(4x4) only)");
  const long long total = (long long)cout * cin * kd;
  const int grid = grid_for(total, 256);
  hipStream_t st = (hipStream_t)stream;
  if (ksize == 2) wino_unpack_kernel<4, 2><<<grid, 256, 0, st>>>(du, dw, cout, cin, rows, cin_pad, kd, total);
  else if (tile == 4) wino_unpack_kernel<4, 3><<<grid, 256, 0, st>>>(du, dw, cout, cin, rows, cin_pad, kd, total);
  else wino_unpack_kernel<2, 3><<<grid, 256, 0, st>>>(du, dw, cout, cin, rows, cin_pad, kd, total);
  CLX_CHECK_LAUNCH("clx_unpack_wgrad_wino");
  return CLX_OK;
}
```

### cellulus_amd/models/plan.py

```python

import ctypes
import math
import os
from dataclasses import dataclass, field
from typing import List, Tuple

import torch

from .. import _clx
from .._clx import ClxConvDesc, ClxSrc


def pad4(c: int) -> int:
    return (c + 3) // 4 * 4


WINO_MIN_CHANNELS = int(os.environ.get("CLX_WINOGRAD_MIN_CHANNELS", "64"))
WINO_TAPS = {1: 16, 2: 36, 3: 36}
WINO_PACK_FWD = {1: 2, 2: 4, 3: 7}
WINO_PACK_DGRAD = {1: 3, 2: 5}
WINO_TILE = {1: 2, 2: 4, 3: 4}


WINO_MIN_CHANNELS_3D = int(os.environ.get("CLX_WINOGRAD_MIN_CHANNELS_3D", "64"))
# ... 806 lines not shown
        src.fz = src.fy = src.fx = 1
        dl.src[0] = src
        dl.B = self.B
        dl.ID, dl.IH, dl.IW = zs
        dl.KD, dl.KH, dl.KW = sp["zk"]
        dl.PD, dl.PH, dl.PW = (k - 1 for k in sp["zk"])
        dl.N = sp["C1p"]
        dl.bias = None
        dl.relu = 0
        dl.accumulate = 0
        dl.algo = 0
        dl.workspace = None
        dl.workspace_bytes = 0
        dl.precision = self.precision
        if dzbuf is not None:
            self._set_mask(dl, up_s.tensor)
        else:
            dl.mask = self.buf[up_s.tensor].data_ptr()
            dl.ld_mask = pad4(low_c)
        dl.out = self.gbuf[up_s.tensor].data_ptr() if dzbuf is not None else None
        dl.ld_out = pad4(low_c)
        return dl

    def _desc(self, layer: ConvLayer):
        d = ClxConvDesc()
        d.nsrc = len(layer.sources)
        t = self.topo
        for i, s in enumerate(layer.sources):
            shape, c = t.shapes[s.tensor]
            src = ClxSrc()
            src.ptr = self.buf[s.tensor].data_ptr()
            src.C = pad4(s.channels)
            src.ld = pad4(c)
            src.D, src.H, src.W = shape
            src.oz, src.oy, src.ox = s.crop
            src.fz, src.fy, src.fx = s.factor
            d.src[i] = src
        d.B = self.B
        d.ID, d.IH, d.IW = layer.in_shape
        d.KD, d.KH, d.KW = layer.kernel
        d.PD = d.PH = d.PW = 0
        d.accumulate = 0
        d.algo = 0
        d.workspace = None
        d.workspace_bytes = 0
        d.precision = self.precision
        d.c_real = layer.sources[0].channels if len(layer.sources) == 1 else 0
        return d

    def _set_gate_out(self, d, name):
        g = getattr(self, "gate", {}).get(name) if self._bwd_ready else None
        if g is not None:
            d.gate_out = g.data_ptr()
            d.ld_gate = g.shape[1]

    def _set_mask(self, d, name, relu=True):
        g = self.gate.get(name)
        if not relu:
            d.mask, d.ld_mask = None, 0
        elif g is not None:
            d.mask, d.ld_mask = None, 0
            d.mask_bits = g.data_ptr()
            d.ld_mask_bits = g.shape[1]
        else:
            d.mask = self.buf[name].data_ptr()
            d.ld_mask = self.buf[name].shape[1]

    def _use_workspace(self, d, code):
        d.algo = code
        if self.workspace is None:
            return
        d.workspace = self.workspace.data_ptr()
        d.workspace_bytes = self.workspace.numel() * 4

    def arena_bytes(self):
        ts = list(self.buf.values()) + [self.workspace, self.aplanes, self.dyplanes, getattr(self, "dyplanes2", None)]
        ts += list(self.xplanes.values()) + list(self.vcache.values())
        return sum(t.numel() * t.element_size() for t in ts if t is not None)

    def _sp_covers(self, d, pass_, algo):
        d.algo = algo
        return bool(_clx.load().clx_conv_sp_covers(ctypes.byref(d), pass_))

    def _decide_sp(self):
        self.sp_pass = {}
        for layer in self.topo.convs:
            if layer.name in self.subpixel:
                self.sp_pass[layer.name] = (False, False, False)
                continue
            a = self.algo[layer.name]
            d = self._desc(layer)
            d.N = layer.cout
            fwd = self._sp_covers(d, 0, a["fwd"])
            d.N = pad4(layer.cout)
            wgrad = self._sp_covers(d, 1, a["wgrad"])
            dgrad = layer.param_index > 0 and self._sp_covers(self._dgrad_desc(layer, None), 0, a["dgrad"])
            self.sp_pass[layer.name] = (fwd, dgrad, wgrad)

    def _register_wplanes(self, wp, k, dgrad=False):
        if wp.data_ptr() not in self._wplanes:
            rows = wp.numel() // k
            nbytes = int(_clx.load().clx_planes_bytes(rows, k))
            self._wplanes[wp.data_ptr()] = (wp, torch.empty(nbytes, dtype=torch.uint8, device=self.device), rows, k, dgrad)

    def _set_wpack(self, d, wp):
        d.wpack = wp.data_ptr()
        e = self._wplanes.get(wp.data_ptr())
        d.wplanes = e[1].data_ptr() if e is not None else None

    def _split_wplanes(self, need_dgrad, st):
        for wp, planes, rows, k, dgrad in self._wplanes.values():
            if need_dgrad or not dgrad:
                _clx.call("clx_split_planes", _clx.ptr(wp), k, rows, k, _clx.ptr(planes), st)

    def _vcache_bytes(self, d, algo, which):
        d.algo = algo
        return int(_clx.load().clx_conv_vcache_bytes(ctypes.byref(d), which))

    def _float_scratch(self, nbytes):
        return torch.empty(nbytes // 4 + 4, dtype=torch.float32, device=self.device)

    def _planes_scratch(self, rows, k):
        return torch.empty(int(_clx.load().clx_planes_bytes(rows, k)), dtype=torch.uint8, device=self.device)

    def _dgrad_desc(self, layer: ConvLayer, dy):
        dd = ClxConvDesc()
        dd.nsrc = 1
        src = ClxSrc()
        src.ptr = dy.data_ptr() if dy is not None else 16
        src.C = pad4(layer.cout)
        src.ld = pad4(layer.cout)
        src.D, src.H, src.W = layer.out_shape
        src.oz = src.oy = src.ox = 0
        src.fz = src.fy = src.fx = 1
        dd.src[0] = src
        dd.B = self.B
        dd.ID, dd.IH, dd.IW = layer.out_shape
        dd.KD, dd.KH, dd.KW = layer.kernel
        dd.PD, dd.PH, dd.PW = (k - 1 for k in layer.kernel)
        dd.N = layer.cin_pad
        dd.bias = None
        dd.relu = 0
        dd.accumulate = 0
        dd.algo = 0
        dd.workspace = None
        dd.workspace_bytes = 0
        dd.precision = self.precision
        return dd

    def _expand_cin(self, layer, w):
        if len(layer.sources) == 1 or all(s.channels % 4 == 0 for s in layer.sources[:-1]):
            return w, layer.cin
        parts, c0 = [], 0
        for s in layer.sources:
            blk = w[:, c0:c0 + s.channels]
            padw = pad4(s.channels) - s.channels
            if padw:
                blk = torch.cat([blk, blk.new_zeros(blk.shape[0], padw, blk.shape[2])], dim=1)
            parts.append(blk)
            c0 += s.channels
        g = torch.cat(parts, dim=1).contiguous()
        return g, g.shape[1]

    def _compress_cin(self, layer, g):
        parts, c0 = [], 0
        for s in layer.sources:
# ... 169 lines not shown
            return None
        special = lambda op: op.name in self.chains or op.name in self.chain_second or op.name in self.subpixel
        first = ops[0]
        if special(first) or len(first.sources) != 1 or first.sources[0].tensor != "raw":
            return None
        readers = tensor_consumers(self.topo)
        tail, src = [], first.out
        for op in ops[1:]:
            if not isinstance(op, ConvLayer) or op.taps != 1 or special(op) or self.algo[op.name]["fwd"]:
                break
            s = op.sources[0]
            if len(op.sources) != 1 or s.tensor != src or tuple(s.crop) != (0, 0, 0) or tuple(s.factor) != (1, 1, 1):
                break
            if readers.get(src, 0) != 1:
                break
            tail.append(op)
            src = op.out
        return (first, tail) if tail else None

    def first_layer_on_rows(self):
        prefix = self.pointwise_prefix()
        if prefix is None or os.environ.get("CLX_SPARSE_FIRST", "1") == "0":
            return False
        first = prefix[0]
        return (self.topo.in_channels == 1 and tuple(first.kernel) in ((1, 3, 3), (3, 3, 3)) and first.cout % 4 == 0
                and first.in_shape[0] >= first.kernel[0])

    def tiled_layer_behind_prefix(self):
        prefix = self.pointwise_prefix()
        if prefix is None:
            return None
        first, tail = prefix
        ops = self.topo.fwd_order
        k = 1 + len(tail)
        if k >= len(ops) or not isinstance(ops[k], ConvLayer):
            return None
        op = ops[k]
        code = self.algo[op.name]["fwd"]
        if (not code or op.kernel[0] != 1 or op.in_shape[0] != 1 or op.name in self.subpixel or op.name in self.chains
                or op.name in self.chain_second or len(op.sources) != 1):
            return None
        s = op.sources[0]
        if s.tensor != tail[-1].out or tuple(s.crop) != (0, 0, 0) or tuple(s.factor) != (1, 1, 1):
            return None
        return op, WINO_TILE[code]

    def _compact(self, slot, rows, width):
        bufs = self.__dict__.setdefault("_compact_bufs", {})
        b = bufs.get(slot)
        if b is None or b.shape[0] < rows or b.shape[1] != width:
            b = bufs[slot] = _clx.zeros((max(rows, 1), width), torch.float32, self.device)
        return b

    def forward_prefix(self, raw, params, nlayers):
        t = self.topo
        st = _clx.stream_ptr(self.device)
        npix_in = t.in_shape[0] * t.in_shape[1] * t.in_shape[2]
        raw = raw.contiguous()
        _clx.call("clx_planar_to_pixel", _clx.ptr(raw), _clx.ptr(self.buf["raw"]), self.B,
                  t.in_channels, npix_in, pad4(t.in_channels), st)
        for op in t.fwd_order[:1 + nlayers]:
            self._conv_forward(op, params, st)
        return self.buf[t.fwd_order[nlayers].out]

    def _conv_forward(self, op, params, st, tiles=None):
        d = self._desc(op)
        d.N = op.cout
        self._set_wpack(d, self.wpack_fwd[op.name])
        b = params[2 * op.param_index + 1]
        d.bias = b.data_ptr() if b is not None else None
        d.relu = 1 if op.relu else 0
        d.mask = None
        d.ld_mask = 0
        d.out = self.buf[op.out].data_ptr()
        d.ld_out = pad4(op.cout)
        if op.relu and self.keep:
            self._set_gate_out(d, op.out)
        if self.sp_pass[op.name][0] and not self.algo[op.name]["fwd"]:
            xp = self.xplanes.get(op.name) if self.keep and self._bwd_ready and tiles is None else None
            d.aplanes = (xp if xp is not None else self.aplanes).data_ptr()
            if xp is not None:
                d.aplanes_valid = 1 if op.name in self._xplanes_fresh else 0
                self._xplanes_fresh.add(op.name)
                nxt = self._pointwise_reader.get(op.out)
                if nxt is not None and os.environ.get("CLX_SP_EPILOGUE_PLANES", "1") != "0":
                    d.out_planes = self.xplanes[nxt.name].data_ptr()
                    self._xplanes_fresh.add(nxt.name)
        if self.algo[op.name]["fwd"]:
            self._use_workspace(d, self.algo[op.name]["fwd"])
            if self.keep and self._bwd_ready and op.name in self.vcache:
                d.vcache = self.vcache[op.name].data_ptr()
                self._vcache_fresh.add(op.name)
            pool = self.fused_pool.get(op.name)
            if pool is not None:
                d.pool_out = self.buf[pool.out].data_ptr()
                d.ld_pool = pad4(pool.channels)
        if tiles is not None:
            d.tile_list = tiles[0].data_ptr()
            d.tile_count = int(tiles[1])
        _clx.call("clx_conv_fwd", ctypes.byref(d), st)

    def _tiles_forward(self, op, params, sparse, st):
        dense = self.buf[op.out]
        clean = sparse["clean_tile_rows"]
        assert clean.shape[1] == dense.shape[1] and clean.shape[0] * self.B == dense.shape[0]
        _clx.call("clx_broadcast_rows", _clx.ptr(clean), clean.numel(), _clx.ptr(dense), self.B, st)
        pool = self.fused_pool.get(op.name)
        if pool is not None:
            pooled, clean_pooled = self.buf[pool.out], sparse["clean_pool_rows"]
            assert clean_pooled.shape[0] * self.B == pooled.shape[0]
            _clx.call("clx_broadcast_rows", _clx.ptr(clean_pooled), clean_pooled.numel(), _clx.ptr(pooled), self.B, st)
        if int(sparse["ntiles"]) > 0:
            self._conv_forward(op, params, st, tiles=(sparse["tiles"], sparse["ntiles"]))

    def _pointwise_on_rows(self, tail, params, sparse, st):
        n, rows = int(sparse["n"]), sparse["rows"]
        src = self.buf[tail[0].sources[0].tensor]
        width = src.shape[1]
        cur = None
        if n > 0:
            cur = self._compact(0, n, width)
            if sparse.get("noisy") is not None:
                first = self.topo.fwd_order[0]
                b = params[2 * first.param_index + 1]
                _clx.call("clx_grey_rows", _clx.ptr(sparse["noisy"]), self.B, *first.in_shape, first.kernel[0],
                          _clx.ptr(rows), n, _clx.ptr(self.wpack_fwd[first.name]), _clx.ptr(b) if b is not None else None,
                          1 if first.relu else 0, first.cout, _clx.ptr(cur), width, st)
            else:
                _clx.call("clx_gather_rows", _clx.ptr(src), width, _clx.ptr(rows), n, width, _clx.ptr(cur), width, st)
            for k, op in enumerate(tail):
                y = self._compact(1 + k % 2, n, pad4(op.cout))
                d = ClxConvDesc()
                d.nsrc = 1
                src_d = ClxSrc()
                src_d.ptr = cur.data_ptr()
                src_d.C = src_d.ld = cur.shape[1]
                src_d.D, src_d.H, src_d.W = 1, 1, n
                src_d.oz = src_d.oy = src_d.ox = 0
                src_d.fz = src_d.fy = src_d.fx = 1
                d.src[0] = src_d
                d.B = 1
                d.ID, d.IH, d.IW = 1, 1, n
                d.KD = d.KH = d.KW = 1
                d.PD = d.PH = d.PW = 0
                d.N = op.cout
                self._set_wpack(d, self.wpack_fwd[op.name])
                d.precision = self.precision
                if self.precision and self.aplanes is not None:
                    d.aplanes = self.aplanes.data_ptr()
                b = params[2 * op.param_index + 1]
                d.bias = b.data_ptr() if b is not None else None
                d.relu = 1 if op.relu else 0
                d.out = y.data_ptr()
                d.ld_out = y.shape[1]
                _clx.call("clx_conv_fwd", ctypes.byref(d), st)
                cur = y
        dense = self.buf[tail[-1].out]
        clean = sparse["clean_rows"]
        assert clean.shape[1] == dense.shape[1] and clean.shape[0] * self.B == dense.shape[0]
        _clx.call("clx_broadcast_rows", _clx.ptr(clean), clean.numel(), _clx.ptr(dense), self.B, st)
        if n > 0:
            _clx.call("clx_scatter_rows", _clx.ptr(cur), cur.shape[1], _clx.ptr(rows), n, dense.shape[1],
                      _clx.ptr(dense), dense.shape[1], st)

    def forward(self, raw, params, out=None, on_op=None, sparse=None):
        t = self.topo
        st = _clx.stream_ptr(self.device)
        sparse_tail = self.pointwise_prefix()[1] if sparse is not None else None
        self._vcache_fresh = set()
        self._xplanes_fresh = set()
        npix_in = t.in_shape[0] * t.in_shape[1] * t.in_shape[2]
        raw = raw.contiguous()
        rows_only_first = sparse is not None and self.first_layer_on_rows()
        if rows_only_first:
            sparse = dict(sparse, noisy=raw)
        else:
            _clx.call("clx_planar_to_pixel", _clx.ptr(raw), _clx.ptr(self.buf["raw"]), self.B,
                      t.in_channels, npix_in, pad4(t.in_channels), st)
        for op_index, op in enumerate(t.fwd_order):
            if on_op is not None and op_index > 0:
                on_op(op_index - 1)
            if op_index == 0 and rows_only_first:
# ... 123 lines not shown
            wtaps = wino_taps(wino_w, layer.kernel) if wino_w else layer.taps
            dwp = self.dwpack[off:off + wtaps * pad4(layer.cout) * layer.cin_pad]
            adjoint = layer.name in self.adjoint
            dual = (self.dycache is not None and wino_w and layer.param_index > 0
                    and self.algo[layer.name]["dgrad"] == wino_w and not adjoint)
            if wino_w:
                self._use_workspace(d, wino_w)
                if layer.name in self.vcache and layer.name in self._vcache_fresh:
                    d.vcache = self.vcache[layer.name].data_ptr()
                    d.vcache_valid = 1
                if dual:
                    d.dy_vcache = self.dycache.data_ptr()
            dy_planes = dy_planes_of.pop(layer.out, None)
            dy_ready = dy_planes is not None
            if dy_planes is None and self.dyplanes is not None:
                dy_planes = self.dyplanes
            if self.sp_pass[layer.name][2] and not wino_w:
                d.aplanes = self.xplanes[layer.name].data_ptr()
                d.aplanes_valid = 1 if layer.name in self._xplanes_fresh else 0
                d.dyplanes = dy_planes.data_ptr()
                d.dyplanes_valid = 1 if dy_ready else 0
                if dy_ready:
                    gb = None
                dy_ready = True
            elif dy_ready:
                raise AssertionError("planes of dY were written for a layer whose weight gradient does not read them")
            self._wgrad(d, dy, pad4(layer.cout), dwp, gb, layer.cout, st)
            yield (layer.param_index,), self._unpack_step(layer, dwp, grads[2 * layer.param_index], wino_w)
            if layer.param_index == 0:
                if dx is not None:
                    self.first_dgrad(layer, dy, params[0], dx, st)
                continue
            dd = self._dgrad_desc(layer, dy)
            self._set_wpack(dd, self.wpack_dgrad[layer.name])
            dgrad_sp = self.sp_pass[layer.name][1] and not self.algo[layer.name]["dgrad"]
            if dgrad_sp:
                dd.aplanes = dy_planes.data_ptr()
                dd.aplanes_valid = 1 if dy_ready else 0
            if self.algo[layer.name]["dgrad"]:
                self._use_workspace(dd, self.algo[layer.name]["dgrad"])
                if adjoint:
                    dd.adjoint = 1
                elif dual:
                    dd.vcache = self.dycache.data_ptr()
                    dd.vcache_valid = 1
            if len(layer.sources) == 2:
                info = r_by_conv0[layer.name]
                cat = self.gbuf["cat%d" % info["level"]]
                dd.mask = None
                dd.ld_mask = 0
                dd.out = cat.data_ptr()
                dd.ld_out = layer.cin_pad
                _clx.call("clx_conv_fwd", ctypes.byref(dd), st)
                skip_s, up_s = layer.sources
                ushape, uc = t.shapes[up_s.tensor]
                LD, LH, LW = layer.in_shape
                _clx.call("clx_upsample_bwd", _clx.ptr(cat), layer.cin_pad, pad4(skip_s.channels),
                          LD, LH, LW, *up_s.crop, _clx.ptr(self.buf[up_s.tensor]),
                          _clx.ptr(self.gbuf[up_s.tensor]), self.B, ushape[0], ushape[1], ushape[2],
                          pad4(uc), *up_s.factor, st)
                pending_skip[skip_s.tensor] = (cat, layer.cin_pad, layer)
            else:
                s = layer.sources[0]
                if s.tensor in pool_by_out:
                    pool = pool_by_out[s.tensor]
                    dd.mask = None
                    dd.ld_mask = 0
                    dd.out = self.gbuf[pool.out].data_ptr()
                    dd.ld_out = pad4(pool.channels)
                    _clx.call("clx_conv_fwd", ctypes.byref(dd), st)
                    cat, ld_cat, rl = pending_skip.pop(pool.src)
                    skip_s = rl.sources[0]
                    D, H, W = pool.in_shape
                    SD, SH, SW = rl.in_shape
                    _clx.call("clx_maxpool_bwd", _clx.ptr(self.buf[pool.src]), _clx.ptr(self.buf[pool.out]),
                              _clx.ptr(self.gbuf[pool.out]), _clx.ptr(cat), ld_cat, SD, SH, SW,
                              *skip_s.crop, _clx.ptr(self.gbuf[pool.src]), self.B, D, H, W,
                              pad4(pool.channels), *pool.factor, st)
                else:
                    prev = by_out[s.tensor]
                    self._set_mask(dd, prev.out, relu=prev.relu)
                    dd.out = self.gbuf[prev.out].data_ptr()
                    dd.ld_out = pad4(prev.cout)
                    if (dgrad_sp and prev.name in self.xplanes and self.sp_pass[prev.name][2]
                            and os.environ.get("CLX_SP_EPILOGUE_PLANES", "1") != "0"):
                        other = self.dyplanes2 if dy_planes is self.dyplanes else self.dyplanes
                        dd.out_planes = other.data_ptr()
                        gbp = grads[2 * prev.param_index + 1]
                        dd.out_colsum = gbp.data_ptr() if gbp is not None else None
                        dy_planes_of[prev.out] = other
                    _clx.call("clx_conv_fwd", ctypes.byref(dd), st)
        assert not pending_skip


def _first_dgrad_kernel_wanted(layer):
    return layer.cin <= 4 and os.environ.get("CLX_FIRST_DGRAD", "1") != "0"


def forward_flops(topo, batch):
    total = 0
    for layer in topo.convs:
        m = batch * layer.out_shape[0] * layer.out_shape[1] * layer.out_shape[2]
        total += 2 * m * layer.cout * layer.cin * layer.taps
    return total


class _Rows:

    def __init__(self, parts, attr):
        self._parts, self._attr = parts, attr

    def __getitem__(self, name):
        return torch.cat([getattr(p, self._attr)[name] for p in self._parts], dim=0)

    def __contains__(self, name):
        return name in getattr(self._parts[0], self._attr)

    def __bool__(self):
        return bool(getattr(self._parts[0], self._attr))

    def get(self, name, default=None):
        return self[name] if name in self else default

    def keys(self):
        return getattr(self._parts[0], self._attr).keys()


def dual_stream_wanted(topo, batch, keep_activations):
    if not keep_activations or batch < 2 or batch % 2 or os.environ.get("CLX_STREAMS", "2") == "1":
        return False
    if os.environ.get("CLX_DETERMINISTIC", "0") == "1":
        return False
    return forward_flops(topo, batch // 2) >= float(os.environ.get("CLX_STREAMS_MIN_GFLOP", "100")) * 1e9


class DualPlan:

    def __init__(self, topo, batch, device, keep_activations):
        assert batch % 2 == 0 and keep_activations
        self.topo, self.B, self.device, self.keep = topo, int(batch), device, True
        self.parts = [UNetPlan(topo, batch // 2, device, True) for _ in range(2)]
        self.streams = [torch.cuda.Stream(device=device) for _ in range(2)]
        self._events = [[], [], []]
        self._shared = False
        self.buf = _Rows(self.parts, "buf")

    def __getattr__(self, name):
        if name in ("parts", "streams"):
            raise AttributeError(name)
        if name == "gbuf":
            return _Rows(self.parts, "gbuf")
        return getattr(self.parts[0], name)

    def pack_weights(self, params, version, need_dgrad):
        a, b = self.parts
        a.pack_weights(params, version, need_dgrad)
        if need_dgrad and not self._shared:
            b._alloc_backward()
            b.share_from(a)
            self._shared = True
        b._packed_version = a._packed_version

    def _fork(self):
        main = torch.cuda.current_stream(self.device)
        for s in self.streams:
            s.wait_stream(main)
        return main

    def _join(self, main):
        for s in self.streams:
            main.wait_stream(s)

    def forward(self, raw, params, out=None):
# ... 83 lines not shown
```

### include/clx.h

```cpp
#ifndef CLX_H
#define CLX_H

#include <stddef.h>
#include <stdint.h>

#ifdef __cplusplus
extern "C" {
#endif

typedef void* clx_stream;

enum clx_status {
  CLX_OK = 0,
  CLX_ERR_ARG = -1,
  CLX_ERR_LAUNCH = -2,
  CLX_ERR_WORKSPACE = -3
};

const char* clx_last_error(void);
int clx_abi_version(void);
int clx_device_count(void);

enum clx_profile_kind {
  CLX_PROF_IGEMM_WIDE = 0,
// ... 15 lines not shown
  CLX_PROF_GEMM_SP2 = 16
};
int clx_profile_enable(int on);
int clx_profile_read(int kind, double* launches, double* total_ms, double* total_flops);
int clx_profile_clock(double* shader_ticks, double* wall_ticks_100mhz, int reset);


typedef struct clx_src {
  const float* ptr;
  int C;
  int ld;
  int D, H, W;
  int oz, oy, ox;
  int fz, fy, fx;
} clx_src;

typedef struct clx_conv_desc {
  int nsrc;
  clx_src src[2];
  int B;
  int ID, IH, IW;
  int KD, KH, KW;
  int PD, PH, PW;
  int N;
  const float* wpack;
  const float* bias;
  int relu;
  const float* mask;
  int ld_mask;
  float* out;
  int ld_out;
  int accumulate;
  int algo;
  void* workspace;
  size_t workspace_bytes;
  void* vcache;
  int vcache_valid;
  int c_real;
  void* dy_vcache;
  unsigned int* gate_out;
  int ld_gate;
  const unsigned int* mask_bits;
  int ld_mask_bits;
  int* det_turns;
  int adjoint;
  float* pool_out;
  int ld_pool;
  const int* tile_list;
  int tile_count;
  int precision;
  const void* wplanes;
  void* aplanes;
  int aplanes_valid;
  void* dyplanes;
  int dyplanes_valid;
  void* out_planes;
  float* out_colsum;
} clx_conv_desc;

enum clx_conv_precision { CLX_PREC_F32 = 0, CLX_PREC_F32X3BF16 = 1 };

enum clx_conv_algo {
  CLX_ALGO_DIRECT = 0,
  CLX_ALGO_WINOGRAD = 1,
  CLX_ALGO_WINOGRAD4 = 2,
  CLX_ALGO_WINOGRAD4_FUSED = 3
};
int clx_conv_fused_applicable(const clx_conv_desc* d);
size_t clx_conv_fused_workspace_bytes(const clx_conv_desc* d);
enum clx_conv_pass { CLX_PASS_FWD = 0, CLX_PASS_WGRAD = 1 };
size_t clx_conv_workspace_bytes(const clx_conv_desc* d, int pass);
size_t clx_conv_vcache_bytes(const clx_conv_desc* d, int which);

size_t clx_planes_bytes(long long rows, int K);
int clx_split_planes(const float* x, long long ld, long long rows, int K, void* planes, clx_stream stream);
int clx_join_planes(const void* planes, long long rows, int K, float* x, long long ld, clx_stream stream);
int clx_gemm_planes(const void* a_planes, const void* b_planes, int M, int N, int K, const float* bias, int relu,
                    float* out, int ld_out, clx_stream stream);
int clx_wgrad_planes(const void* dy_planes, const void* x_planes, long long rows, int N, int C, float* dw, int ld_dw,
                     clx_stream stream);

int clx_conv_sp_covers(const clx_conv_desc* d, int pass);

int clx_conv_fwd(const clx_conv_desc* d, clx_stream stream);

size_t clx_conv_wgrad_turns_bytes(const clx_conv_desc* d);
size_t clx_colsum_scratch_bytes(int N);
int clx_colsum_ordered(const float* x, int ld, long long M, int N, float* out, void* scratch, clx_stream stream);

int clx_chain64_fwd(const float* x, int ld_x, long long M, const float* w1, const float* b1, float* y1,
                    int ld_y1, unsigned int* gate1, int ld_gate1, const float* w2, const float* b2, int N2,
                    int relu2, float* y2, int ld_y2, unsigned int* gate2, int ld_gate2, clx_stream stream);
int clx_chain64_bwd(const float* dp2, int ld_dp2, int N2, const float* y1, int ld_y1, const float* x,
                    int ld_x, int gate_x, long long M, const float* w2t, const float* w1t, float* dp0,
                    int ld_dp0, float* dw2, float* db2, float* dw1, float* db1, clx_stream stream);

int clx_conv_wgrad(const clx_conv_desc* d, const float* dy, int ld_dy,
                   float* dwpack, float* dbias, clx_stream stream);

enum clx_pack_mode {
  CLX_PACK_FWD = 0,
  CLX_PACK_DGRAD = 1,
  CLX_PACK_WINO_FWD = 2,
  CLX_PACK_WINO_DGRAD = 3,
  CLX_PACK_WINO4_FWD = 4,
  CLX_PACK_WINO4_DGRAD = 5,
  CLX_PACK_WINO4_ADJOINT = 6,
  CLX_PACK_WINO4_FUSED = 7
};
int clx_pack_weights(const float* w, float* wp, int cout, int cin, int taps,
                     int cin_pad, int cout_pad, int mode, clx_stream stream);
typedef struct clx_pack_job {
  const float* w;
  float* wp;
  int cout, cin, taps, cin_pad, cout_pad, mode;
} clx_pack_job;
int clx_pack_weights_batch(const clx_pack_job* jobs, int njobs, long long max_total, clx_stream stream);
int clx_unpack_wgrad(const float* dwpack, float* dw, int cout, int cin, int taps,
                     int rows, int cin_pad, clx_stream stream);
int clx_unpack_wgrad_wino(const float* du, float* dw, int cout, int cin, int rows,
                          int cin_pad, int tile, int ksize, int kd, clx_stream stream);

int clx_planar_to_pixel(const float* planar, float* pixel, int B, int C,
                        long long n, int ld, clx_stream stream);
int clx_pixel_to_planar(const float* pixel, float* planar, int B, int C,
                        long long n, int ld, clx_stream stream);

int clx_depth_to_space(const float* lo, int ld_lo, float* hi, int ld_hi, int B, int D, int H,
                       int W, int N, int fz, int fy, int fx, clx_stream stream);
int clx_space_to_depth(const float* hi, int ld_hi, float* lo, int ld_lo, int B, int D, int H,
                       int W, int N, int fz, int fy, int fx, clx_stream stream);

int clx_subpixel_split_weights(const float* w, float* w_skip, float* weff, int cout, int cin,
                               int C0, int N, int kd, int kh, int kw, int fz, int fy, int fx,
                               clx_stream stream);
int clx_subpixel_fold_grads(const float* g_skip, const float* g_eff, float* gw, int cout, int cin,
                            int C0, int N, int kd, int kh, int kw, int fz, int fy, int fx,
                            clx_stream stream);

int clx_maxpool_fwd(const float* x, float* y, int B, int D, int H, int W, int C,
                    int fz, int fy, int fx, clx_stream stream);
int clx_maxpool_bwd(const float* x, const float* y, const float* dy_pool,
                    const float* dskip, int ld_skip, int SD, int SH, int SW,
                    int cz, int cy, int cx, float* dx, int B, int D, int H,
                    int W, int C, int fz, int fy, int fx, clx_stream stream);
int clx_upsample_bwd(const float* dcat, int ld_cat, int coff, int LD, int LH,
                     int LW, int oz, int oy, int ox, const float* y, float* dy,
                     int B, int D, int H, int W, int C, int fz, int fy, int fx,
                     clx_stream stream);

int clx_gather_add_fwd(const float* offsets, const long long* coords, float* sel,
                       int B, int P, int ND, int Z, int Y, int X, int* oob_count,
                       clx_stream stream);
int clx_gather_add_bwd(const float* dsel, const long long* coords, float* doffsets,
                       int B, int P, int ND, int Z, int Y, int X, int* oob_count,
                       clx_stream stream);
int clx_oce_loss_fwd_bwd(const float* a, const float* r, float* da, double* sums,
                         long long npairs, int ND, float temperature,
                         float reg_weight, float grad_scale, clx_stream stream);
int clx_oce_pairs_fused(const float* offsets, const long long* anchor,
                        const long long* reference, float* doffsets, double* sums,
                        int B, int P, int ND, int Z, int Y, int X,
                        float temperature, float reg_weight, clx_stream stream);
size_t clx_oce_pairs_det_scratch_bytes(int B, int ND, long long npix);
int clx_oce_pairs_fused_det(const float* offsets, const long long* anchor, const long long* reference,
                            float* doffsets, double* sums, int B, int P, int ND, int Z, int Y, int X,
// ... 151 lines not shown
```

Measured before the change: 310.9.

## Write split-precision planes from Winograd and small-channel conv epilogues

Extends the producer-side epilogue that writes bf16 split planes (and bias-gradient column sums) to the Winograd forward and adjoint data-gradient output kernels and to the small-channel grey kernel. Before, only the split-precision 1x1 product could do this. The next 1x1 consumer or weight-gradient pass can then skip a separate split pass over the activation or gradient. When nothing else reads the fp32 data gradient, the fp32 output is dropped entirely. In exchange the epilogues gain extra stores, shared-memory atomics for the column sums, and a reduced launch bound.

```diff
diff --git a/cellulus_amd/_clx.py b/cellulus_amd/_clx.py
--- a/cellulus_amd/_clx.py
+++ b/cellulus_amd/_clx.py
@@ -112,6 +112,7 @@
     "clx_conv_workspace_bytes": (c_size_t, [POINTER(ClxConvDesc), _I]),
     "clx_conv_vcache_bytes": (c_size_t, [POINTER(ClxConvDesc), _I]),
     "clx_conv_sp_covers": (_I, [POINTER(ClxConvDesc), _I]),
+    "clx_conv_writes_planes": (_I, [POINTER(ClxConvDesc)]),
     "clx_planes_bytes": (c_size_t, [_LL, _I]),
     "clx_split_planes": (_I, [_P, _LL, _LL, _I, _P, _P]),
     "clx_join_planes": (_I, [_P, _LL, _I, _P, _LL, _P]),
diff --git a/cellulus_amd/csrc/clx_common.h b/cellulus_amd/csrc/clx_common.h
--- a/cellulus_amd/csrc/clx_common.h
+++ b/cellulus_amd/csrc/clx_common.h
@@ -54,6 +54,7 @@
 static inline int cdiv(long long a, long long b) { return (int)((a + b - 1) / b); }
 
 bool clx_smallc_applicable(const clx_conv_desc* d);
+bool clx_smallc_writes_planes(const clx_conv_desc* d);
 int clx_smallc_fwd(const clx_conv_desc* d, hipStream_t st);
 int clx_smallc_wgrad(const clx_conv_desc* d, const float* dy, int ld_dy, float* dwpack,
                      float* dbias, hipStream_t st);
@@ -66,6 +67,7 @@
 bool clx_sp_wgrad_rule(const clx_conv_desc* d);
 bool clx_sp_applicable(const clx_conv_desc* d);
 bool clx_wino_sp(const clx_conv_desc* d);
+bool clx_wino_writes_planes(const clx_conv_desc* d);
 int clx_sp_launch(const void* A, const void* B, int M, int N, int K, long long rows_a, int batch, long long bs_a, long long bs_b,
                   long long bs_out, const clx_conv_desc* ep, hipStream_t st);
 int clx_sp_clock_read(double* shader_ticks, double* wall_ticks, int reset);
diff --git a/cellulus_amd/csrc/conv_igemm.hip b/cellulus_amd/csrc/conv_igemm.hip
--- a/cellulus_amd/csrc/conv_igemm.hip
+++ b/cellulus_amd/csrc/conv_igemm.hip
@@ -565,7 +565,14 @@
 extern "C" int clx_conv_fwd(const clx_conv_desc* d, clx_stream stream) {
   int rc = conv_validate(d, "clx_conv_fwd");
   if (rc) return rc;
-  CLX_REQUIRE(d->wpack && d->out, "clx_conv_fwd: null wpack/out");
+  const bool sp_product = d->algo == CLX_ALGO_DIRECT && d->aplanes != nullptr && clx_sp_applicable(d);
+  const bool wino_planes = (d->algo == CLX_ALGO_WINOGRAD || d->algo == CLX_ALGO_WINOGRAD4) && d->workspace != nullptr &&
+                           d->tile_list == nullptr && clx_wino_writes_planes(d);
+  const bool grey_planes = d->algo == CLX_ALGO_DIRECT && clx_smallc_writes_planes(d) && d->mask == nullptr &&
+                           d->mask_bits == nullptr && d->gate_out == nullptr;
+  CLX_REQUIRE(d->wpack != nullptr, "clx_conv_fwd: null wpack");
+  CLX_REQUIRE(d->out != nullptr || (d->out_planes != nullptr && !d->accumulate && (sp_product || (wino_planes && d->adjoint))),
+              "clx_conv_fwd: null out (only a data gradient that writes out_planes, without accumulate, may leave it out)");
   CLX_REQUIRE(d->N > 0 && d->ld_out >= d->N, "clx_conv_fwd: bad N/ld_out");
   CLX_REQUIRE(((uintptr_t)d->wpack & 15) == 0, "clx_conv_fwd: wpack must be 16-byte aligned");
   CLX_REQUIRE(d->mask == nullptr || (d->ld_mask >= d->N && d->ld_mask % 4 == 0 &&
@@ -580,16 +587,19 @@
   CLX_REQUIRE(d->algo == CLX_ALGO_DIRECT || d->algo == CLX_ALGO_WINOGRAD || d->algo == CLX_ALGO_WINOGRAD4 ||
                   d->algo == CLX_ALGO_WINOGRAD4_FUSED,
               "clx_conv_fwd: bad algo");
-  CLX_REQUIRE((d->out_planes == nullptr && d->out_colsum == nullptr && !d->aplanes_valid) ||
-                  (d->algo == CLX_ALGO_DIRECT && d->aplanes != nullptr && clx_sp_applicable(d)),
+  CLX_REQUIRE((d->out_planes == nullptr && d->out_colsum == nullptr && !d->aplanes_valid) || sp_product ||
+                  (!d->aplanes_valid && d->out_planes != nullptr &&
+                   ((wino_planes && (d->adjoint || d->out_colsum == nullptr)) || (grey_planes && d->out_colsum == nullptr))),
               "clx_conv_fwd: out_planes / out_colsum / aplanes_valid need the split-precision 1x1 product "
-              "(clx_conv_sp_covers, wplanes and aplanes)");
+              "(clx_conv_sp_covers, wplanes and aplanes); out_planes alone also a producer clx_conv_writes_planes names, "
+              "out_colsum with it the adjoint Winograd data gradient");
   if (d->algo == CLX_ALGO_WINOGRAD4_FUSED) return clx_wino_fused_fwd(d, (hipStream_t)stream);
   if (d->algo != CLX_ALGO_DIRECT) return clx_wino_fwd(d, (hipStream_t)stream);
   CLX_REQUIRE(d->pool_out == nullptr && d->tile_list == nullptr && !d->adjoint,
               "clx_conv_fwd: pool_out / tile_list / adjoint need a Winograd algorithm (algo = %d)", d->algo);
   if (clx_smallc_applicable(d) && d->mask == nullptr && d->mask_bits == nullptr && d->gate_out == nullptr) {
-    clx_smallc_fwd(d, (hipStream_t)stream);
+    rc = clx_smallc_fwd(d, (hipStream_t)stream);
+    if (rc) return rc;
     CLX_CHECK_LAUNCH("clx_conv_fwd(small-channel)");
     return CLX_OK;
   }
@@ -597,6 +607,16 @@
   if (rc) return rc;
   CLX_CHECK_LAUNCH("clx_conv_fwd");
   return CLX_OK;
+}
+
+extern "C" int clx_conv_writes_planes(const clx_conv_desc* d) {
+  if (d == nullptr) return 0;
+  const int both = CLX_PLANES_OUT | CLX_PLANES_COLSUM;
+  if (d->algo == CLX_ALGO_DIRECT)
+    return d->adjoint ? 0 : clx_sp_fwd_rule(d) ? both : clx_smallc_writes_planes(d) ? CLX_PLANES_OUT : 0;
+  if (d->algo == CLX_ALGO_WINOGRAD || d->algo == CLX_ALGO_WINOGRAD4)
+    return !clx_wino_writes_planes(d) ? 0 : d->adjoint ? both : CLX_PLANES_OUT;
+  return 0;
 }
 
 int clx_igemm_launch(const clx_conv_desc* d, int batch, long long bs_in, long long bs_w,
diff --git a/cellulus_amd/csrc/conv_smallc.hip b/cellulus_amd/csrc/conv_smallc.hip
--- a/cellulus_amd/csrc/conv_smallc.hip
+++ b/cellulus_amd/csrc/conv_smallc.hip
@@ -1,4 +1,5 @@
 #include "clx_common.h"
+#include "sp_planes.h"
 
 namespace {
 
@@ -13,6 +14,7 @@
   const float* bias;
   float* out;
   int ld_out, relu;
+  char* out_planes;
   const float* dy;
   int ld_dy;
   float* dwp;
@@ -264,7 +266,7 @@
   }
 };
 
-template <int KD>
+template <int KD, bool PL = false>
 __global__ __launch_bounds__(256) void conv_grey_fwd_kernel(const SmallP p) {
   using L = GreyLane<KD>;
   const L ln(p);
@@ -304,8 +306,10 @@
 #pragma unroll
         for (int e = 0; e < 4; ++e) acc[e] = fmaxf(acc[e], 0.f);
       }
-      if (live_n && r[s].ox0 + ln.px < p.OW)
+      if (live_n && r[s].ox0 + ln.px < p.OW) {
         *reinterpret_cast<f32x4*>(p.out + (size_t)(r[s].m0 + ln.px) * p.ld_out + n) = acc;
+        if constexpr (PL) sp::store4(p.out_planes, r[s].m0 + ln.px, n, p.N >> 4, acc);
+      }
       item += stride;
     }
   }
@@ -473,12 +477,25 @@
   return taps > 1 && taps <= MAX_TAPS && d->N >= 4;
 }
 
+bool clx_smallc_writes_planes(const clx_conv_desc* d) {
+  return clx_smallc_applicable(d) && d->N % 16 == 0 && d->ld_out % 4 == 0;
+}
+
 int clx_smallc_fwd(const clx_conv_desc* d, hipStream_t st) {
   SmallP p{};
   fill(d, p);
   p.wpack = d->wpack; p.bias = d->bias; p.out = d->out; p.ld_out = d->ld_out; p.relu = d->relu;
+  CLX_REQUIRE(d->out_planes == nullptr || clx_smallc_writes_planes(d), "clx_conv_fwd(small-channel): out_planes needs N %% 16 == 0");
   if (grey_applicable(d, d->ld_out) && ((uintptr_t)d->out & 15) == 0 && (!d->bias || ((uintptr_t)d->bias & 15) == 0)) {
     const dim3 grid = grey_grid(p);
+    if (d->out_planes != nullptr) {
+      const int rc = clx_sp_zero_tail(d->out_planes, p.M, p.N, 1, 0, st);
+      if (rc) return rc;
+      p.out_planes = (char*)d->out_planes;
+      if (d->KD == 1) conv_grey_fwd_kernel<1, true><<<grid, 256, 0, st>>>(p);
+      else conv_grey_fwd_kernel<3, true><<<grid, 256, 0, st>>>(p);
+      return CLX_OK;
+    }
     if (d->KD == 1) conv_grey_fwd_kernel<1><<<grid, 256, 0, st>>>(p);
     else conv_grey_fwd_kernel<3><<<grid, 256, 0, st>>>(p);
     return CLX_OK;
@@ -496,6 +513,7 @@
     case 32: conv_smallc_fwd_kernel<32><<<grid, 256, lds, st>>>(p); break;
     default: conv_smallc_fwd_kernel<64><<<grid, 256, lds, st>>>(p); break;
   }
+  if (d->out_planes != nullptr) return clx_sp_split(d->out, d->ld_out, p.M, p.N, d->out_planes, nullptr, 0, st);
   return CLX_OK;
 }
 
diff --git a/cellulus_amd/csrc/gemm_sp.hip b/cellulus_amd/csrc/gemm_sp.hip
--- a/cellulus_amd/csrc/gemm_sp.hip
+++ b/cellulus_amd/csrc/gemm_sp.hip
@@ -222,9 +222,11 @@
 #pragma unroll
         for (int e = 0; e < 4; ++e) val[j][e] = (!live[j] || mk[j][e] > 0.f) ? val[j][e] : 0.f;
     }
-#pragma unroll
-    for (int j = 0; j < PH; ++j)
-      if (live[j]) *reinterpret_cast<f32x4*>(out_base + (size_t)mrow[j] * p.ld_out) = val[j];
+    if (p.out) {
+#pragma unroll
+      for (int j = 0; j < PH; ++j)
+        if (live[j]) *reinterpret_cast<f32x4*>(out_base + (size_t)mrow[j] * p.ld_out) = val[j];
+    }
     if (p.out_planes) {
 #pragma unroll
       for (int j = 0; j < PH; ++j)
@@ -1180,6 +1182,7 @@
   p.out_planes = batch == 1 ? (char*)ep->out_planes : nullptr;
   p.colsum = batch == 1 ? ep->out_colsum : nullptr; p.colsum_n = N;
   CLX_REQUIRE(p.out_planes == nullptr || ep->ld_out == N, "clx_gemm_planes: out_planes needs a dense output (ld_out == N)");
+  CLX_REQUIRE(p.out != nullptr || (p.out_planes != nullptr && !p.accumulate), "clx_gemm_planes: a null out needs out_planes and no accumulate");
   p.nbm = cdiv(M, SP_BM); p.nbn = N / SP_BN;
   const char* const tile_env = getenv("CLX_SP_TILE");
   const int tile_choice = tile_env != nullptr ? atoi(tile_env) : 0;
diff --git a/cellulus_amd/csrc/wino.hip b/cellulus_amd/csrc/wino.hip
--- a/cellulus_amd/csrc/wino.hip
+++ b/cellulus_amd/csrc/wino.hip
@@ -90,7 +90,7 @@
   }
 }
 
-template <int MT, int R>
+template <int MT, int R, bool PL = false>
 __global__ __launch_bounds__(256) void wino_output_kernel(const float* __restrict__ M, int N4, Geom g,
                                                           const float* __restrict__ bias, int relu,
                                                           const float* __restrict__ mask, int ld_mask,
@@ -99,17 +99,25 @@
                                                           int ld_gate, const unsigned int* __restrict__ mask_bits,
                                                           int ld_mask_bits, float* __restrict__ pool_out, int ld_pool,
                                                           long long total, const int* __restrict__ tile_list = nullptr,
-                                                          long long Tc = 0) {
+                                                          long long Tc = 0, char* __restrict__ planes = nullptr) {
   using W = WT<MT, R>;
   constexpr int A = W::A;
   constexpr int MP = MT / 2;
   const int N = N4 * 4;
-  const long long plane = (tile_list ? Tc : g.T) * N;
+  const long long Trows = tile_list ? Tc : g.T;
+  const long long plane = Trows * N;
   const int sub = threadIdx.x & 7;
   for (long long i = (long long)blockIdx.x * blockDim.x + threadIdx.x; i < total;
        i += (long long)gridDim.x * blockDim.x) {
-    const int n = (int)(i % N4) * 4;
-    const long long t = i / N4;
+    int n;
+    long long t;
+    if constexpr (PL) {
+      sp::item_to_row_channel(i, N, t, n);
+      if (t >= Trows) continue;
+    } else {
+      n = (int)(i % N4) * 4;
+      t = i / N4;
+    }
     const long long tg = tile_list ? (long long)tile_list[t] : t;
     const int tx = (int)(tg % g.tw);
     const long long q = tg / g.tw;
@@ -180,6 +188,7 @@
             for (int e = 0; e < 4; ++e) v[e] = (mk[e] > 0.f) ? v[e] : 0.f;
           }
           st4(out + m * ld_out + n, v);
+          if constexpr (PL) sp::store4(planes, m, n, N >> 4, v);
         } else {
           for (int e = 0; e < 4 && n + e < Nreal; ++e) {
             float xv = v[e];
@@ -205,21 +214,38 @@
 
 constexpr int ADJ_SEG = 8;
 
-__global__ __launch_bounds__(256) void wino_adjoint_output_kernel(const float* __restrict__ Pm, int C4, int Bn, int th,
+template <bool PL = false, bool FM = false>
+__global__ __launch_bounds__(256, 2) void wino_adjoint_output_kernel(const float* __restrict__ Pm, int C4, int Bn, int th,
                                                                   int tw, int IH, int IW, const float* __restrict__ mask,
                                                                   int ld_mask, const unsigned int* __restrict__ mask_bits,
                                                                   int ld_mask_bits, float* __restrict__ out, int ld_out,
-                                                                  int Creal, long long total) {
+                                                                  int Creal, long long total, char* __restrict__ planes = nullptr,
+                                                                  float* __restrict__ colsum = nullptr) {
   using W = WT<4, 3>;
   constexpr int A = 6;
+  extern __shared__ float bacc[];
   const int C = C4 * 4;
   const int bh = (IH + 3) / 4, bw = (IW + 3) / 4;
   const int nseg = (bh + ADJ_SEG - 1) / ADJ_SEG;
   const long long plane = (long long)Bn * th * tw * C;
+  if constexpr (PL) {
+    if (colsum) {
+      for (int k = threadIdx.x; k < C; k += blockDim.x) bacc[k] = 0.f;
+      __syncthreads();
+    }
+  }
   for (long long i = (long long)blockIdx.x * blockDim.x + threadIdx.x; i < total;
        i += (long long)gridDim.x * blockDim.x) {
-    const int c = (int)(i % C4) * 4;
-    long long t = i / C4;
+    int c;
+    long long t;
+    if constexpr (PL) {
+      sp::item_to_row_channel(i, C, t, c);
+      if (t >= (long long)Bn * nseg * bw) continue;
+    } else {
+      c = (int)(i % C4) * 4;
+      t = i / C4;
+    }
+    f32x4 csum = {0.f, 0.f, 0.f, 0.f};
     const int bx = (int)(t % bw);
     long long q = t / bw;
     const int sg = (int)(q % nseg);
@@ -285,7 +311,16 @@
 #pragma unroll
               for (int k = 0; k < 4; ++k) v[k] = ((wbits >> k) & 1u) ? v[k] : 0.f;
             }
-            if (c + 3 < Creal) {
+            if constexpr (PL) {
+              if constexpr (FM) {
+                const f32x4 mk = ld4(mask + m * ld_mask + c);
+#pragma unroll
+                for (int k = 0; k < 4; ++k) v[k] = (mk[k] > 0.f) ? v[k] : 0.f;
+              }
+              if (out) st4(out + m * ld_out + c, v);
+              sp::store4(planes, m, c, C >> 4, v);
+              csum += v;
+            } else if (c + 3 < Creal) {
               if (mask) {
                 const f32x4 mk = ld4(mask + m * ld_mask + c);
 #pragma unroll
@@ -304,6 +339,19 @@
       }
 #pragma unroll
       for (int e = 0; e < 4; ++e) { carry[0][e] = d[4][e]; carry[1][e] = d[5][e]; }
+    }
+    if constexpr (PL) {
+      if (colsum) {
+#pragma unroll
+        for (int e = 0; e < 4; ++e) atomicAdd(&bacc[c + e], csum[e]);
+      }
+    }
+  }
+  if constexpr (PL) {
+    if (colsum) {
+      __syncthreads();
+      for (int k = threadIdx.x; k < Creal; k += blockDim.x)
+        if (bacc[k] != 0.f) atomicAdd(colsum + k, bacc[k]);
     }
   }
 }
@@ -744,9 +792,22 @@
                     d->mask == nullptr && d->mask_bits == nullptr && !d->accumulate,
                 "clx_conv_fwd(winograd): pool_out needs N %% 4 == 0, an aligned ld_pool >= N, and no mask / accumulate");
   }
+  if (d->out_planes != nullptr) {
+    const long long rows = (long long)gout.B * gout.OH * gout.OW;
+    CLX_REQUIRE(clx_wino_writes_planes(d) && list == nullptr && rows < (1ll << 31),
+                "clx_conv_fwd(winograd): out_planes needs a 2-D layer with N %% 32 == 0, no tile_list and fewer than 2^31 pixels");
+    const int rc = clx_sp_zero_tail(d->out_planes, rows, Np, 1, 0, st);
+    if (rc) return rc;
+    const long long tot_pl = sp_items(Tout, Np);
+    CLX_LAUNCH_KIND(CLX_PROF_WINO_TRANSFORM, (wino_output_kernel<MT, R, true>), dim3(grid_for(tot_pl, 256)), dim3(256), 0, st, M, Np / 4, gout,
+                    d->bias, d->relu, d->mask, d->ld_mask, d->out, d->ld_out, d->N, d->accumulate, d->gate_out, d->ld_gate, d->mask_bits,
+                    d->ld_mask_bits, d->pool_out, d->ld_pool, tot_pl, list, Tout, (char*)d->out_planes);
+    CLX_CHECK_LAUNCH("clx_conv_fwd(winograd, planes)");
+    return CLX_OK;
+  }
   CLX_LAUNCH_KIND(CLX_PROF_WINO_TRANSFORM, (wino_output_kernel<MT, R>), dim3(grid_for(tot_out, 256)), dim3(256), 0, st, M, Np / 4, gout, d->bias,
                   d->relu, d->mask, d->ld_mask, d->out, d->ld_out, d->N, d->accumulate, d->gate_out, d->ld_gate, d->mask_bits,
-                  d->ld_mask_bits, d->pool_out, d->ld_pool, tot_out, list, Tout);
+                  d->ld_mask_bits, d->pool_out, d->ld_pool, tot_out, list, Tout, (char*)nullptr);
   CLX_CHECK_LAUNCH("clx_conv_fwd(winograd)");
   return CLX_OK;
 }
@@ -832,6 +893,12 @@
 
 bool clx_wino_sp(const clx_conv_desc* d) { return wino_sp(d); }
 
+bool clx_wino_writes_planes(const clx_conv_desc* d) {
+  if (d->N <= 0 || d->N % 32 != 0) return false;
+  if (d->adjoint) return d->algo == CLX_ALGO_WINOGRAD4;
+  return applicable(d) && d->KD == 1;
+}
+
 extern "C" size_t clx_conv_workspace_bytes(const clx_conv_desc* d, int pass) {
   if (d == nullptr || !applicable(d)) return 0;
   if (pass == CLX_PASS_WGRAD && d->PH != 0) return 0;
@@ -878,6 +945,10 @@
               "clx_conv_fwd(adjoint): needs the %zu workspace bytes of the layer's weight gradient (%zu given)", need,
               d->workspace_bytes);
   CLX_REQUIRE(d->mask_bits == nullptr || Cp % 32 == 0, "clx_conv_fwd(adjoint): mask_bits needs whole words per pixel");
+  const long long rows_dx = (long long)d->B * planes_dx * (OHf + 2) * (OWf + 2);
+  CLX_REQUIRE(d->out_planes == nullptr ||
+                  (clx_wino_writes_planes(d) && rows_dx < (1ll << 31) && (d->out == nullptr || d->ld_out >= Cp)),
+              "clx_conv_fwd(adjoint): out_planes needs a channel count that is a multiple of 32 and fewer than 2^31 pixels");
   float* P = (float*)d->workspace;
   float* Mdy = P + (size_t)36 * Tdx * Cp;
   if (spx) {
@@ -902,9 +973,28 @@
   }
   const int IH = OHf + 2, IW = OWf + 2;
   const int nseg = ((IH + 3) / 4 + ADJ_SEG - 1) / ADJ_SEG;
-  const long long total = (long long)d->B * planes_dx * nseg * ((IW + 3) / 4) * (Cp / 4);
-  CLX_LAUNCH_KIND(CLX_PROF_WINO_TRANSFORM, wino_adjoint_output_kernel, dim3(grid_for(total, 256)), dim3(256), 0, st, P, Cp / 4,
-                  d->B * planes_dx, th, tw, IH, IW, d->mask, d->ld_mask, d->mask_bits, d->ld_mask_bits, d->out, d->ld_out, Cp, total);
+  const long long cols = (long long)d->B * planes_dx * nseg * ((IW + 3) / 4);
+  if (d->out_planes != nullptr) {
+    const int rc = clx_sp_zero_tail(d->out_planes, rows_dx, Cp, 1, 0, st);
+    if (rc) return rc;
+    const long long total = sp_items(cols, Cp);
+    int blocks = grid_for(total, 256);
+    if (d->out_colsum && blocks > 2048) blocks = 2048;
+    if (d->mask != nullptr)
+      CLX_LAUNCH_KIND(CLX_PROF_WINO_TRANSFORM, (wino_adjoint_output_kernel<true, true>), dim3(blocks), dim3(256), (size_t)Cp * sizeof(float),
+                      st, P, Cp / 4, d->B * planes_dx, th, tw, IH, IW, d->mask, d->ld_mask, d->mask_bits, d->ld_mask_bits, d->out,
+                      d->ld_out, Cp, total, (char*)d->out_planes, d->out_colsum);
+    else
+      CLX_LAUNCH_KIND(CLX_PROF_WINO_TRANSFORM, (wino_adjoint_output_kernel<true, false>), dim3(blocks), dim3(256), (size_t)Cp * sizeof(float),
+                      st, P, Cp / 4, d->B * planes_dx, th, tw, IH, IW, d->mask, d->ld_mask, d->mask_bits, d->ld_mask_bits, d->out,
+                      d->ld_out, Cp, total, (char*)d->out_planes, d->out_colsum);
+    CLX_CHECK_LAUNCH("clx_conv_fwd(winograd adjoint, planes)");
+    return CLX_OK;
+  }
+  const long long total = cols * (Cp / 4);
+  CLX_LAUNCH_KIND(CLX_PROF_WINO_TRANSFORM, (wino_adjoint_output_kernel<false, false>), dim3(grid_for(total, 256)), dim3(256), 0, st, P, Cp / 4,
+                  d->B * planes_dx, th, tw, IH, IW, d->mask, d->ld_mask, d->mask_bits, d->ld_mask_bits, d->out, d->ld_out, Cp, total,
+                  (char*)nullptr, (float*)nullptr);
   CLX_CHECK_LAUNCH("clx_conv_fwd(winograd adjoint)");
   return CLX_OK;
 }
diff --git a/cellulus_amd/models/plan.py b/cellulus_amd/models/plan.py
--- a/cellulus_amd/models/plan.py
+++ b/cellulus_amd/models/plan.py
@@ -912,6 +912,14 @@
         d.algo = algo
         return bool(_clx.load().clx_conv_sp_covers(ctypes.byref(d), pass_))
 
+    @staticmethod
+    def _writes_planes(d, colsum=False):
+        return bool(_clx.load().clx_conv_writes_planes(ctypes.byref(d)) & (2 if colsum else 1))
+
+    @staticmethod
+    def _producer_planes():
+        return os.environ.get("CLX_SP_EPILOGUE_PLANES", "1") != "0"
+
     def _decide_sp(self):
         self.sp_pass = {}
         for layer in self.topo.convs:
@@ -1247,10 +1255,6 @@
             if xp is not None:
                 d.aplanes_valid = 1 if op.name in self._xplanes_fresh else 0
                 self._xplanes_fresh.add(op.name)
-                nxt = self._pointwise_reader.get(op.out)
-                if nxt is not None and os.environ.get("CLX_SP_EPILOGUE_PLANES", "1") != "0":
-                    d.out_planes = self.xplanes[nxt.name].data_ptr()
-                    self._xplanes_fresh.add(nxt.name)
         if self.algo[op.name]["fwd"]:
             self._use_workspace(d, self.algo[op.name]["fwd"])
             if self.keep and self._bwd_ready and op.name in self.vcache:
@@ -1263,6 +1267,11 @@
         if tiles is not None:
             d.tile_list = tiles[0].data_ptr()
             d.tile_count = int(tiles[1])
+        nxt = self._pointwise_reader.get(op.out)
+        if (nxt is not None and self.keep and self._bwd_ready and tiles is None and self._producer_planes()
+                and self._writes_planes(d)):
+            d.out_planes = self.xplanes[nxt.name].data_ptr()
+            self._xplanes_fresh.add(nxt.name)
         _clx.call("clx_conv_fwd", ctypes.byref(d), st)
 
     def _tiles_forward(self, op, params, sparse, st):
@@ -1552,13 +1561,16 @@
                     self._set_mask(dd, prev.out, relu=prev.relu)
                     dd.out = self.gbuf[prev.out].data_ptr()
                     dd.ld_out = pad4(prev.cout)
-                    if (dgrad_sp and prev.name in self.xplanes and self.sp_pass[prev.name][2]
-                            and os.environ.get("CLX_SP_EPILOGUE_PLANES", "1") != "0"):
+                    if (prev.name in self.xplanes and self.sp_pass[prev.name][2] and self._producer_planes()
+                            and self._writes_planes(dd, colsum=True)):
                         other = self.dyplanes2 if dy_planes is self.dyplanes else self.dyplanes
                         dd.out_planes = other.data_ptr()
                         gbp = grads[2 * prev.param_index + 1]
                         dd.out_colsum = gbp.data_ptr() if gbp is not None else None
                         dy_planes_of[prev.out] = other
+                        if (prev.param_index > 0 and self.sp_pass[prev.name][1] and not self.algo[prev.name]["dgrad"]
+                                and not self.deterministic):
+                            dd.out = None
                     _clx.call("clx_conv_fwd", ctypes.byref(dd), st)
         assert not pending_skip
 
diff --git a/include/clx.h b/include/clx.h
--- a/include/clx.h
+++ b/include/clx.h
@@ -121,6 +121,9 @@
 
 int clx_conv_sp_covers(const clx_conv_desc* d, int pass);
 
+enum clx_planes_support { CLX_PLANES_OUT = 1, CLX_PLANES_COLSUM = 2 };
+int clx_conv_writes_planes(const clx_conv_desc* d);
+
 int clx_conv_fwd(const clx_conv_desc* d, clx_stream stream);
 
 size_t clx_conv_wgrad_turns_bytes(const clx_conv_desc* d);
```

Result: no change. 308.8 (-0.7%).
